# urgent-challenge/urgent2026_challenge_track1

Hardware: NVIDIA B200
Metric: BSRNN audio-sec/sec enhanced at 48 kHz (higher is better)
Workload: dtype fp16

## Files before the change

### include/bsrnn_b200.h

```cpp
#ifndef BSRNN_B200_H_
#define BSRNN_B200_H_

#include <stdint.h>
#include <stddef.h>

#ifdef __cplusplus
extern "C" {
#endif

const char* bsrnn_last_error(void);
int bsrnn_abi_version(void);
int bsrnn_device_check(void);
long bsrnn_launch_count(int reset);

int bsrnn_fft_twiddle(float* twiddle, int n_fft, void* stream);
int bsrnn_stft_fwd(const float* wav, const int32_t* lens, float* spec, const float* twiddle, int B, int L,
                   int n_fft, int hop, int transform, float exponent, float factor, void* stream);

int bsrnn_istft_fwd(const float* spec, const float* mask, const float* resid, float* spec_out, float* wav_out,
                    const float* twiddle, int B, int T, int L_out, int n_fft, int hop, int transform,
                    float exponent, float factor, void* stream);

int bsrnn_gn_stats(const float* x, double* stats, int B, long rows_per_sample, int C, long row_stride, void* stream);
int bsrnn_band_stats(const float* x, double* stats, int B, int T, long row_len, const int32_t* band_off,
                     const int32_t* band_width, int n_bands, void* stream);
int bsrnn_gn_finalize(const double* stats, const float* gamma, const float* beta, const float* extra,
                      float* scale, float* shift, int G, int C, const double* counts, float eps, int G_inner,
                      void* stream);

typedef struct {
  const float* A; const float* W; const float* bias; float* C;
  const float* scale; const float* shift;
  long a_inner, a_outer_stride, a_inner_stride;
  long c_inner, c_outer_stride, c_inner_stride;
  long rows_per_sample, ss_stride;
  int M, N, K, k_valid, ldw, epilogue, n_store, pad_;
} bsrnn_gemm_desc;
int bsrnn_gemm_f32(const bsrnn_gemm_desc* descs, int n_groups, int max_m, int max_n, void* stream);

int bsrnn_blstm_recurrence_f32(const float* gates_x, const float* w_hh, float* y, float* c_state,
                               int R, int steps, int H, long seq_inner, long seq_outer, long seq_inner_stride,
                               long step_stride, void* stream);

int bsrnn_norm_cast_kb8(const float* x, const float* scale, const float* shift, void* out, long ldx, int col0, int C,
                        int kcores, int m_tiles, int tiles_per_step, int R, long seq_inner, long seq_outer,
                        long seq_inner_stride, long step_stride, long tokens_per_sample, int g_inner, void* stream);
int bsrnn_norm_cast_kb8_ones(const float* x, const float* scale, const float* shift, void* out, long ldx, int col0,
                             int C, int kcores, int m_tiles, int tiles_per_step, int R, long seq_inner, long seq_outer,
                             long seq_inner_stride, long step_stride, long tokens_per_sample, int g_inner, int one_col,
                             void* stream);
int bsrnn_gemm_tc(const void* A, const void* W, const float* bias, void* out, double* stats, int m_tiles, int n_tiles,
                  int kcores, int BN, int epilogue, long ldo, int n_valid, int out_kcores, long tokens_per_sample,
                  int tiles_per_step, int R, long seq_inner, long seq_outer, long seq_inner_stride, long step_stride,
                  void* stream);
int bsrnn_gemm_tc_ex(const void* A, const void* W, const float* bias, void* out, double* stats, int m_tiles, int n_tiles,
                     int kcores, int BN, int epilogue, long ldo, int n_valid, int out_kcores, long tokens_per_sample,
                     int tiles_per_step, int R, long seq_inner, long seq_outer, long seq_inner_stride, long step_stride,
                     int stats_inner, int flags, void* stream);
int bsrnn_gemm_tc_grouped(const void* A, const void* W, const float* bias, void* out, double* stats,
                          const long long* groups, int n_groups, int m_tiles, int kc_max, int BN, long ldo, int n_valid,
                          long tokens_per_sample, int tiles_per_step, int R, long seq_inner, long seq_outer,
                          long seq_inner_stride, long step_stride, void* stream);
int bsrnn_gemm_tc_limit_ctas(int n);
int bsrnn_band_norm_cast_kb8(const float* spec, const float* scale, const float* shift, void* out, const int32_t* c_off,
                             const int32_t* bin0, const int32_t* width2, const long long* a_off, int K, long rows, int T,
                             int F2, int cmax, void* stream);
int bsrnn_lstm_step_tc(const void* A, const void* W, const void* gx, float* cstate, void* out_h, int m_tiles, int n_tiles,
                       int BN, int H, long ld_gx, void* stream);
int bsrnn_blstm_step_tc(const void* A_f, const void* W_f, const void* gx_f, float* c_f, void* out_f, const void* A_b,
                        const void* W_b, const void* gx_b, float* c_b, void* out_b, int m_tiles, int n_tiles, int BN,
                        int H, long ld_gx, void* stream);
int bsrnn_blstm_recurrence_tc(const void* gates_x, const void* w_pack, const void* zero_tile, void* y, int R, int steps,
                              int seq_tiles, int max_clusters, void* stream);
int bsrnn_blstm_recurrence_tc_ex(const void* gates_x, const void* w_pack, const void* zero_tile, void* y, int R,
                                 int steps, int seq_tiles, int max_clusters, int slots, void* stream);
int bsrnn_blstm_tc_max_clusters(void);
int bsrnn_blstm_tc_max_pair_clusters(void);
int bsrnn_blstm_recurrence_tc_flag(const void* gates_x, const void* w_pack, const void* zero_tile, void* y, int R,
                                   int steps, int seq_tiles, int max_groups, int slots, void* sync_ws, void* stream);
int bsrnn_blstm_tc_flag_max_groups(void);
int bsrnn_blstm_tc_sync_bytes(void);
int bsrnn_blstm_fused_tc(const void* xhat, const void* w_fused, const void* zero_tile, void* y, int R, int steps,
                         int seq_tiles, int max_groups, int slots, void* sync_ws, void* stream);
int bsrnn_blstm_fused_max_groups(void);
int bsrnn_blstm_fused_sync_bytes(void);
int bsrnn_blstm_fused7_tc(const void* xhat, const void* w_fused7, const void* zero_tile, void* y, int R, int steps,
                          int seq_tiles, int max_groups, int slots, void* sync_ws, void* stream);
int bsrnn_blstm_fused7_max_groups(void);
int bsrnn_blstm_fused14_tc(const void* xhat, const void* w_fused14, const void* zero_tile, void* y, int R, int steps,
                           int seq_tiles, int max_groups, int slots, void* sync_ws, void* stream);
int bsrnn_blstm_fused_train_tc(int geo, const void* xhat, const void* w_fused, const void* zero_tile, void* y_f, void* y_b,
                               long y_stride, void* gates, float* c_f, float* c_b, void* scratch, int R, int steps,
                               int seq_tiles, int max_groups, int slots, void* sync_ws, void* stream);
long bsrnn_blstm_fused_train_scratch_bytes(int steps, int seq_tiles);
int bsrnn_blstm_fused14_max_groups(void);
int bsrnn_blstm_fused768_tc(const void* xhat, const void* w_fused, const void* zero_tile, void* y_f, void* y_b,
                            long y_stride, int R, int steps, int seq_tiles, int max_groups, int slots, void* sync_ws,
                            void* stream);
int bsrnn_blstm_fused768_max_groups(void);

void bsrnn_debug_set_lstm_schedule(int ver);

int bsrnn_blstm_train_fwd_f32(const float* gates_x, const float* w_hh, float* y, float* c_state, float* saved, int R,
                              int steps, int H, long seq_inner, long seq_outer, long seq_inner_stride,
                              long step_stride, void* stream);
int bsrnn_blstm_train_bwd_f32(const float* dy, const float* saved, const float* w_hh, float* dgates, float* dh_rec,
                              float* dc_carry, int R, int steps, int H, long seq_inner, long seq_outer,
                              long seq_inner_stride, long step_stride, void* stream);
int bsrnn_grad_sumsq(const float* grad, long n, double* stats, void* stream);
int bsrnn_adamw_step(float* param, const float* grad, float* exp_avg, float* exp_avg_sq, float* ema, long n,
                     const double* stats, float grad_scale, float max_norm, float lr, float beta1, float beta2,
                     float eps, float weight_decay, int step, float ema_decay, void* stream);
int bsrnn_adamw_step2(float* param, const float* grad, float* exp_avg, float* exp_avg_sq, float* ema, long n,
                      double* state, const long* skip_ranges, int n_skip, float grad_scale, float max_norm, float lr,
                      float beta1, float beta2, float eps, float weight_decay, float ema_decay, void* stream);

int bsrnn_blstm_step_train_tc(const void* A_f, const void* W_f, void* gx_f, const float* cprev_f, float* cout_f, void* out_f,
                              const void* A_b, const void* W_b, void* gx_b, const float* cprev_b, float* cout_b,
                              void* out_b, int m_tiles, int n_tiles, int BN, int H, long ld_gx, void* stream);
int bsrnn_blstm_bwd_step_tc(const void* A_f, const void* W_f, const void* sg_f, const void* dy_f, const float* ccur_f,
                            const float* cprev_f, float* dc_f, void* out_f, const void* A_b, const void* W_b,
                            const void* sg_b, const void* dy_b, const float* ccur_b, const float* cprev_b, float* dc_b,
                            void* out_b, int m_tiles, int n_tiles, int BN, int H, long ld_sg, long ld_dy, int valid_rows,
                            void* stream);
int bsrnn_blstm_train_fwd_tc(const void* zero_tile, void* y_f, void* y_b, const void* W_f, const void* W_b, void* gates,
                             float* c_f, float* c_b, int steps, int tiles, int n_tiles, int BN, int H, void* stream);
int bsrnn_blstm_train_bwd_tc(const void* zero_tile, void* dG_f, void* dG_b, const void* WT_f, const void* WT_b,
                             const void* gates, const void* dy, const float* c_f, const float* c_b, float* dc_f, float* dc_b,
                             int steps, int tiles, int n_tiles, int BN, int H, int valid_rows, void* stream);
int bsrnn_gemm_tc_scaled(const void* A, const void* W, const float* bias, void* out, int m_tiles, int n_tiles, int kcores,
                         int BN, long ldo, int n_valid, float out_scale, const float* out_scale_ptr, int ksplit,
                         int tiles_per_step, int R, long seq_inner, long seq_outer, long seq_inner_stride,
                         long step_stride, void* stream);
int bsrnn_kb8_transpose(const void* src, void* dst, int src_m0, int m_count, int kc_src, int BN, int n_tiles,
                        long dst_kcores, long dst_kc0, void* stream);

int bsrnn_stft_stats_fwd(const float* wav, const int32_t* lens, float* spec, const float* twiddle, int B, int L, int n_fft,
                         int hop, int transform, float exponent, float factor, double* band_stats,
                         const int32_t* band_bin0, int n_bands, void* stream);
int bsrnn_band_split_fwd(const float* spec, const float* scale, const float* shift, const float* wT, const float* bias,
                         float* out, const int32_t* c_off, const int32_t* bin0, const int32_t* width2,
                         const int32_t* c_off_host, int K, long rows, int T, int F2, int N, int cmax, long ldo,
                         int out_width, int out_col, void* stream);

int bsrnn_istft_bwd(const float* d_wav, float* d_spec, const float* twiddle, int B, int T, int L_out, int n_fft, int hop,
                    void* stream);

int bsrnn_l1_time_fwd_bwd(const float* est, const float* tgt, double* loss, float* grad, int B, int L, float weight,
                          void* stream);
int bsrnn_mrl1_spec_fwd_bwd(const float* est, const float* tgt, double* loss, float* grad, const float* twiddle, int B,
                            int L, int window, float weight, void* stream);

int bsrnn_time_embed(const float* t, const float* W, float* out, int B, int E, void* stream);
int bsrnn_conv5x5_glu(const float* g, const float* weight, const float* bias, float* out, int B, int T, int Fp,
                      int F, void* stream);
int bsrnn_euler_step(float* x, const float* mask, const float* resid, float step, long n_complex, void* stream);
int bsrnn_axpy_complex(float* out, const float* y, const float* z, float sigma, long n_complex, void* stream);
int bsrnn_complex_mask(float* out, const float* x, const float* mask, const float* resid, float sign, long n_complex,
                       void* stream);

#ifdef __cplusplus
}
#endif
#endif
```

### urgent2026_challenge_track1_b200/_lib.py

```python
from __future__ import annotations

import ctypes as C
import os

import numpy as np
import torch

_HERE = os.path.dirname(os.path.abspath(__file__))
LIB_PATH = os.path.join(_HERE, "_C", "libbsrnn_b200.so")

c_void_p, c_int, c_long, c_float, c_double = C.c_void_p, C.c_int, C.c_long, C.c_float, C.c_double

PROTOTYPES = {
    "bsrnn_abi_version": [],
    "bsrnn_device_check": [],
    "bsrnn_launch_count": [c_int],
    "bsrnn_fft_twiddle": [c_void_p, c_int, c_void_p],
    "bsrnn_stft_fwd": [c_void_p, c_void_p, c_void_p, c_void_p, c_int, c_int, c_int, c_int, c_int, c_float, c_float,
                       c_void_p],
    "bsrnn_istft_fwd": [c_void_p, c_void_p, c_void_p, c_void_p, c_void_p, c_void_p, c_int, c_int, c_int, c_int,
                        c_int, c_int, c_float, c_float, c_void_p],
    "bsrnn_gn_stats": [c_void_p, c_void_p, c_int, c_long, c_int, c_long, c_void_p],
    "bsrnn_band_stats": [c_void_p, c_void_p, c_int, c_int, c_long, c_void_p, c_void_p, c_int, c_void_p],
    "bsrnn_gn_finalize": [c_void_p, c_void_p, c_void_p, c_void_p, c_void_p, c_void_p, c_int, c_int, c_void_p,
                          c_float, c_int, c_void_p],
    "bsrnn_gemm_f32": [c_void_p, c_int, c_int, c_int, c_void_p],
    "bsrnn_blstm_recurrence_f32": [c_void_p, c_void_p, c_void_p, c_void_p, c_int, c_int, c_int, c_long, c_long,
                                   c_long, c_long, c_void_p],
    "bsrnn_norm_cast_kb8": [c_void_p, c_void_p, c_void_p, c_void_p, c_long, c_int, c_int, c_int, c_int, c_int, c_int,
                            c_long, c_long, c_long, c_long, c_long, c_int, c_void_p],
    "bsrnn_norm_cast_kb8_ones": [c_void_p, c_void_p, c_void_p, c_void_p, c_long, c_int, c_int, c_int, c_int, c_int,
                                 c_int, c_long, c_long, c_long, c_long, c_long, c_int, c_int, c_void_p],
    "bsrnn_gemm_tc": [c_void_p, c_void_p, c_void_p, c_void_p, c_void_p, c_int, c_int, c_int, c_int, c_int, c_long,
                      c_int, c_int, c_long, c_int, c_int, c_long, c_long, c_long, c_long, c_void_p],
    "bsrnn_gemm_tc_ex": [c_void_p, c_void_p, c_void_p, c_void_p, c_void_p, c_int, c_int, c_int, c_int, c_int, c_long,
                         c_int, c_int, c_long, c_int, c_int, c_long, c_long, c_long, c_long, c_int, c_int, c_void_p],
    "bsrnn_gemm_tc_grouped": [c_void_p, c_void_p, c_void_p, c_void_p, c_void_p, c_void_p, c_int, c_int, c_int, c_int, c_long,
                              c_int, c_long, c_int, c_int, c_long, c_long, c_long, c_long, c_void_p],
    "bsrnn_gemm_tc_limit_ctas": [c_int],
    "bsrnn_blstm_fused_train_tc": [c_int, c_void_p, c_void_p, c_void_p, c_void_p, c_void_p, c_long, c_void_p, c_void_p, c_void_p,
                                   c_void_p, c_int, c_int, c_int, c_int, c_int, c_void_p, c_void_p],
    "bsrnn_blstm_fused_train_scratch_bytes": [c_int, c_int],
    "bsrnn_band_norm_cast_kb8": [c_void_p, c_void_p, c_void_p, c_void_p, c_void_p, c_void_p, c_void_p, c_void_p, c_int,
                                 c_long, c_int, c_int, c_int, c_void_p],
    "bsrnn_lstm_step_tc": [c_void_p, c_void_p, c_void_p, c_void_p, c_void_p, c_int, c_int, c_int, c_int, c_long, c_void_p],
    "bsrnn_blstm_step_tc": [c_void_p, c_void_p, c_void_p, c_void_p, c_void_p, c_void_p, c_void_p, c_void_p, c_void_p, c_void_p,
                            c_int, c_int, c_int, c_int, c_long, c_void_p],
    "bsrnn_blstm_recurrence_tc": [c_void_p, c_void_p, c_void_p, c_void_p, c_int, c_int, c_int, c_int, c_void_p],
    "bsrnn_blstm_recurrence_tc_ex": [c_void_p, c_void_p, c_void_p, c_void_p, c_int, c_int, c_int, c_int, c_int,
                                     c_void_p],
    "bsrnn_blstm_recurrence_tc_flag": [c_void_p, c_void_p, c_void_p, c_void_p, c_int, c_int, c_int, c_int, c_int,
                                       c_void_p, c_void_p],
    "bsrnn_blstm_fused_tc": [c_void_p, c_void_p, c_void_p, c_void_p, c_int, c_int, c_int, c_int, c_int, c_void_p, c_void_p],
    "bsrnn_blstm_fused768_tc": [c_void_p, c_void_p, c_void_p, c_void_p, c_void_p, c_long, c_int, c_int, c_int, c_int, c_int,
                                c_void_p, c_void_p],
    "bsrnn_blstm_fused768_max_groups": [],
    "bsrnn_blstm_fused7_tc": [c_void_p, c_void_p, c_void_p, c_void_p, c_int, c_int, c_int, c_int, c_int, c_void_p, c_void_p],
    "bsrnn_blstm_fused7_max_groups": [],
    "bsrnn_blstm_fused14_tc": [c_void_p, c_void_p, c_void_p, c_void_p, c_int, c_int, c_int, c_int, c_int, c_void_p, c_void_p],
    "bsrnn_blstm_fused14_max_groups": [],
    "bsrnn_blstm_fused_max_groups": [],
    "bsrnn_blstm_fused_sync_bytes": [],
    "bsrnn_blstm_tc_flag_max_groups": [],
    "bsrnn_blstm_tc_sync_bytes": [],
    "bsrnn_blstm_tc_max_clusters": [],
    "bsrnn_blstm_tc_max_pair_clusters": [],
    "bsrnn_debug_set_lstm_schedule": [c_int],
    "bsrnn_blstm_train_fwd_f32": [c_void_p, c_void_p, c_void_p, c_void_p, c_void_p, c_int, c_int, c_int, c_long, c_long,
                                  c_long, c_long, c_void_p],
    "bsrnn_blstm_train_bwd_f32": [c_void_p, c_void_p, c_void_p, c_void_p, c_void_p, c_void_p, c_int, c_int, c_int,
                                  c_long, c_long, c_long, c_long, c_void_p],
    "bsrnn_grad_sumsq": [c_void_p, c_long, c_void_p, c_void_p],
    "bsrnn_adamw_step": [c_void_p, c_void_p, c_void_p, c_void_p, c_void_p, c_long, c_void_p, c_float, c_float, c_float,
                         c_float, c_float, c_float, c_float, c_int, c_float, c_void_p],
    "bsrnn_adamw_step2": [c_void_p, c_void_p, c_void_p, c_void_p, c_void_p, c_long, c_void_p, c_void_p, c_int, c_float,
                          c_float, c_float, c_float, c_float, c_float, c_float, c_float, c_void_p],
    "bsrnn_blstm_step_train_tc": [c_void_p] * 12 + [c_int, c_int, c_int, c_int, c_long, c_void_p],
    "bsrnn_blstm_bwd_step_tc": [c_void_p] * 16 + [c_int, c_int, c_int, c_int, c_long, c_long, c_int, c_void_p],
    "bsrnn_blstm_train_fwd_tc": [c_void_p] * 8 + [c_int, c_int, c_int, c_int, c_int, c_void_p],
    "bsrnn_blstm_train_bwd_tc": [c_void_p] * 11 + [c_int, c_int, c_int, c_int, c_int, c_int, c_void_p],
    "bsrnn_gemm_tc_scaled": [c_void_p, c_void_p, c_void_p, c_void_p, c_int, c_int, c_int, c_int, c_long, c_int, c_float,
                             c_void_p, c_int, c_int, c_int, c_long, c_long, c_long, c_long, c_void_p],
    "bsrnn_kb8_transpose": [c_void_p, c_void_p, c_int, c_int, c_int, c_int, c_int, c_long, c_long, c_void_p],
    "bsrnn_stft_stats_fwd": [c_void_p, c_void_p, c_void_p, c_void_p, c_int, c_int, c_int, c_int, c_int, c_float, c_float,
                             c_void_p, c_void_p, c_int, c_void_p],
    "bsrnn_band_split_fwd": [c_void_p] * 10 + [c_int, c_long, c_int, c_int, c_int, c_int, c_long, c_int, c_int, c_void_p],
    "bsrnn_istft_bwd": [c_void_p, c_void_p, c_void_p, c_int, c_int, c_int, c_int, c_int, c_void_p],
    "bsrnn_l1_time_fwd_bwd": [c_void_p, c_void_p, c_void_p, c_void_p, c_int, c_int, c_float, c_void_p],
    "bsrnn_mrl1_spec_fwd_bwd": [c_void_p, c_void_p, c_void_p, c_void_p, c_void_p, c_int, c_int, c_int, c_float, c_void_p],
    "bsrnn_time_embed": [c_void_p, c_void_p, c_void_p, c_int, c_int, c_void_p],
    "bsrnn_conv5x5_glu": [c_void_p, c_void_p, c_void_p, c_void_p, c_int, c_int, c_int, c_int, c_void_p],
    "bsrnn_euler_step": [c_void_p, c_void_p, c_void_p, c_float, c_long, c_void_p],
    "bsrnn_axpy_complex": [c_void_p, c_void_p, c_void_p, c_float, c_long, c_void_p],
    "bsrnn_complex_mask": [c_void_p, c_void_p, c_void_p, c_void_p, c_float, c_long, c_void_p],
}

GEMM_DESC = np.dtype([
    ("A", "<u8"), ("W", "<u8"), ("bias", "<u8"), ("C", "<u8"), ("scale", "<u8"), ("shift", "<u8"),
    ("a_inner", "<i8"), ("a_outer_stride", "<i8"), ("a_inner_stride", "<i8"),
    ("c_inner", "<i8"), ("c_outer_stride", "<i8"), ("c_inner_stride", "<i8"),
    ("rows_per_sample", "<i8"), ("ss_stride", "<i8"),
    ("M", "<i4"), ("N", "<i4"), ("K", "<i4"), ("k_valid", "<i4"), ("ldw", "<i4"), ("epilogue", "<i4"),
    ("n_store", "<i4"), ("pad_", "<i4"),
])
assert GEMM_DESC.itemsize == 144

EPI_STORE, EPI_TANH, EPI_RESIDUAL, EPI_GLU = 0, 1, 2, 3
TC_F16_ROWS, TC_RESID_F32, TC_TANH_KB8, TC_GLU_F32, TC_F16_KB8 = 0, 1, 2, 3, 4
TC_TANH_F32 = 7
TC_RESID_TMA = 8

_lib = None


class NativeLibraryError(RuntimeError):
    pass


def lib():
    global _lib
    if _lib is None:
        if not os.path.exists(LIB_PATH):
            raise NativeLibraryError(
                f"{LIB_PATH} not found: the CUDA extension is not built (run ./build.sh). "
                "There is no CPU or PyTorch fallback for this path.")
        handle = C.CDLL(LIB_PATH)
        for name, argtypes in PROTOTYPES.items():
            fn = getattr(handle, name)
            fn.argtypes = argtypes
            fn.restype = c_int
        handle.bsrnn_launch_count.restype = C.c_long
        handle.bsrnn_blstm_fused_train_scratch_bytes.restype = C.c_long
        handle.bsrnn_last_error.restype = C.c_char_p
        handle.bsrnn_last_error.argtypes = []
        _lib = handle
    return _lib


def check(rc: int, what: str):
    if rc != 0:
        raise RuntimeError(f"{what} failed (rc={rc}): {lib().bsrnn_last_error().decode()}")


_DEVICE_OK = set()


def require_device():
    if not torch.cuda.is_available():
        raise NativeLibraryError("no CUDA device: the B200 path has no CPU fallback")
    dev = torch.cuda.current_device()
    if dev not in _DEVICE_OK:
        check(lib().bsrnn_device_check(), "bsrnn_device_check")
        _DEVICE_OK.add(dev)


def ptr(t):
    if t is None:
        return None
    return t.data_ptr()


def stream_ptr():
    return torch.cuda.current_stream().cuda_stream


def call(name, *args):
    check(getattr(lib(), name)(*args), name)
```

### urgent2026_challenge_track1_b200/csrc/gemm_tc.cu

```cuda
#include "common.cuh"
#include "umma.cuh"
#include "tmap.cuh"
#include <cuda_fp16.h>
#include <stdlib.h>

namespace bsrnn {
using namespace umma;

constexpr int TC_STAGES = 8;
constexpr int TC_KS = 8;
constexpr int TC_EPI_WARPS = 8;
#ifndef BSRNN_RESID_EPI_WARPS
#define BSRNN_RESID_EPI_WARPS 12
#endif
__host__ __device__ constexpr int tc_epi_warps(int epi) { return (epi == 1  || epi == 8 ) ? BSRNN_RESID_EPI_WARPS : TC_EPI_WARPS; }
__host__ __device__ constexpr int tc_threads(int epi) { return (2 + tc_epi_warps(epi)) * 32; }
constexpr int TC_SCR_LD = 36;
constexpr int TC_SCR_BYTES = tc_epi_warps(1) * 32 * TC_SCR_LD * 4;
constexpr int TC_ACC_COLS = 256;

struct RowMap {
  int tiles_per_step;
  int R;
  long seq_inner, seq_outer, seq_inner_stride, step_stride;
  __device__ __forceinline__ bool map(int m_tile, int r, long* token) const {
    const int step = m_tile / tiles_per_step;
    const int j = m_tile - step * tiles_per_step;
    const int seq = j * 128 + r;
    if (seq >= R) return false;
    if (seq_inner == 1) *token = (long)seq * seq_outer + (long)step * step_stride;
    else if (seq_inner >= (long)R) *token = (long)seq * seq_inner_stride + (long)step * step_stride;
    else {
      const int si = (int)seq_inner, q = seq / si;
      *token = (long)q * seq_outer + (long)(seq - q * si) * seq_inner_stride + (long)step * step_stride;
    }
    return true;
  }
};

struct GemmTcArgs {
  const __half* A;
  const __half* W;
  const float* bias;
  void* out;
  double* stats;
  long ldo;
  long tokens_per_sample;
  int m_tiles, n_tiles, kcores, BN;
  int n_valid;
  int out_kcores;
  int b_resident;
  int pf_dist;
  int ks;
  const __half* gx;
  float* cstate;
  long ld_gx;
  int H;
  int dir_tiles;
  const __half* A2; const __half* W2; const __half* gx2; float* cstate2; void* out2;
  int debug;
  int stages;
  RowMap rows;
  float out_scale;
  const float* out_scale_ptr;
  int ksplit, kps, m_log;
  int mc;
  int save_gates;
  float* cstate_out; float* cstate_out2;
  const __half* dy; const __half* dy2;
  long ld_dy;
  const float* c_cur; const float* c_cur2;
  const float* c_prev; const float* c_prev2;
  int valid_rows;
  alignas(64) CUtensorMap tmap;
  const long long* groups;
  int n_groups;
  int l2_keep;
  int reverse_m;
  int m_inner;
  int use_tmap;
  int tm_col_step;
  int run_merge;
  int no_resid;
  int stats_inner;
};

enum { EPI_F16_ROWS = 0, EPI_RESID_F32 = 1, EPI_TANH_KB8 = 2, EPI_GLU_F32 = 3, EPI_F16_KB8 = 4, EPI_LSTM_STEP = 5,
       EPI_LSTM_BWD = 6, EPI_TANH_F32 = 7, EPI_RESID_TMA = 8 };

__device__ __forceinline__ float fast_tanh(float x) {
  float y;
  asm("tanh.approx.f32 %0, %1;" : "=f"(y) : "f"(x));
  return y;
}
__device__ __forceinline__ float fast_sigmoid(float x) { return fmaf(fast_tanh(0.5f * x), 0.5f, 0.5f); }

__device__ __forceinline__ uint32_t pack_h2(float a, float b) {
  __half2 v = __floats2half2_rn(a, b);
  return *reinterpret_cast<uint32_t*>(&v);
}

struct BwdSub {
  uint4 g[4];
  uint4 dy;
  float4 cc[2], cq[2], dc[2];
};
__device__ __forceinline__ void bwd_load(BwdSub& R, const __half* sgp, const __half* dyp, const float* ccp, const float* cpp,
                                         const float* dcp, int b8) {
#pragma unroll
  for (int i = 0; i < 4; ++i) R.g[i] = __ldg(reinterpret_cast<const uint4*>(sgp + 32 * b8) + i);
  R.dy = __ldg(reinterpret_cast<const uint4*>(dyp + 8 * b8));
  R.cc[0] = __ldg(reinterpret_cast<const float4*>(ccp + 8 * b8));
  R.cc[1] = __ldg(reinterpret_cast<const float4*>(ccp + 8 * b8 + 4));
  R.cq[0] = R.cq[1] = make_float4(0.f, 0.f, 0.f, 0.f);
  if (cpp) {
    R.cq[0] = __ldg(reinterpret_cast<const float4*>(cpp + 8 * b8));
    R.cq[1] = __ldg(reinterpret_cast<const float4*>(cpp + 8 * b8 + 4));
  }
  R.dc[0] = *reinterpret_cast<const float4*>(dcp + 8 * b8);
  R.dc[1] = *reinterpret_cast<const float4*>(dcp + 8 * b8 + 4);
}
__device__ __forceinline__ void bwd_unit(float dh_rec, float dy, float i_, float f_, float g_, float o_, float ct, float cprev,
                                         float& dc_carry, uint32_t& w0, uint32_t& w1) {
  const float dh = dy + dh_rec;
  const float tc = fast_tanh(ct);
  const float d_o = dh * tc;
  const float dc = dc_carry + dh * o_ * (1.f - tc * tc);
  const float d_i = dc * g_, d_g = dc * i_, d_f = dc * cprev;
  dc_carry = dc * f_;
  w0 = pack_h2(d_i * i_ * (1.f - i_), d_f * f_ * (1.f - f_));
  w1 = pack_h2(d_g * (1.f - g_ * g_), d_o * o_ * (1.f - o_));
}
__device__ __forceinline__ void bwd_compute(BwdSub& R, float a0, float a1, float a2, float a3, float a4, float a5, float a6,
                                            float a7, uint32_t (&dgw)[16]) {
  const __half2* gh = reinterpret_cast<const __half2*>(R.g);
  const __half2* dyh = reinterpret_cast<const __half2*>(&R.dy);
  const float acc[8] = {a0, a1, a2, a3, a4, a5, a6, a7};
  const float ct[8] = {R.cc[0].x, R.cc[0].y, R.cc[0].z, R.cc[0].w, R.cc[1].x, R.cc[1].y, R.cc[1].z, R.cc[1].w};
  const float cp[8] = {R.cq[0].x, R.cq[0].y, R.cq[0].z, R.cq[0].w, R.cq[1].x, R.cq[1].y, R.cq[1].z, R.cq[1].w};
  float dcs[8] = {R.dc[0].x, R.dc[0].y, R.dc[0].z, R.dc[0].w, R.dc[1].x, R.dc[1].y, R.dc[1].z, R.dc[1].w};
#pragma unroll
  for (int j = 0; j < 8; ++j) {
    const float2 g_if = __half22float2(gh[2 * j]), g_go = __half22float2(gh[2 * j + 1]);
    const float2 d2 = __half22float2(dyh[j >> 1]);
    bwd_unit(acc[j], (j & 1) ? d2.y : d2.x, g_if.x, g_if.y, g_go.x, g_go.y, ct[j], cp[j], dcs[j], dgw[2 * j], dgw[2 * j + 1]);
  }
  R.dc[0] = make_float4(dcs[0], dcs[1], dcs[2], dcs[3]);
  R.dc[1] = make_float4(dcs[4], dcs[5], dcs[6], dcs[7]);
}

template <int EPI, int NC>
__device__ __forceinline__ void epilogue_chunk(const GemmTcArgs& a, int m, int n, int r, int c0, const uint32_t* acc,
                                               bool row_ok, long token, float& s_sum, float& s_sq, float* scr, int lane,
                                               float bias_lane) {
  const int gc0 = n * a.BN + c0;
  float v[NC];
  if (a.bias) {
#pragma unroll
    for (int i = 0; i < NC; ++i) v[i] = __uint_as_float(acc[i]) + __shfl_sync(0xffffffffu, bias_lane, i);
  } else {
#pragma unroll
    for (int i = 0; i < NC; ++i) v[i] = __uint_as_float(acc[i]);
  }
  if (EPI == EPI_RESID_F32 && (a.out_scale != 0.f || a.out_scale_ptr)) {
    const float sc = a.out_scale_ptr ? __ldg(a.out_scale_ptr) : a.out_scale;
#pragma unroll
    for (int i = 0; i < NC; ++i) v[i] *= sc;
  }

  if (EPI == EPI_F16_ROWS) {
    if (!row_ok) return;
    __half* o = reinterpret_cast<__half*>(a.out) + token * a.ldo + gc0;
#pragma unroll
    for (int i = 0; i < NC; i += 8) {
      uint4 pk = make_uint4(pack_h2(v[i], v[i + 1]), pack_h2(v[i + 2], v[i + 3]), pack_h2(v[i + 4], v[i + 5]),
                            pack_h2(v[i + 6], v[i + 7]));
      *reinterpret_cast<uint4*>(o + i) = pk;
    }
  } else if (EPI == EPI_RESID_F32) {
    if (a.debug & 4) return;
    float* my = scr + (r & 31) * TC_SCR_LD;
#pragma unroll
    for (int i = 0; i < NC; i += 4) *reinterpret_cast<float4*>(my + i) = make_float4(v[i], v[i + 1], v[i + 2], v[i + 3]);
    __syncwarp();
    const int sub = lane >> 3, c4 = (lane & 7) * 4;
    const unsigned okmask = __ballot_sync(0xffffffffu, row_ok);
    const bool col_ok = c4 < NC && gc0 + c4 + 3 < a.n_valid;
    float* optr[8];
    float4 old[8];
#pragma unroll
    for (int i = 0; i < 8; ++i) {
      const int rr = 4 * i + sub;
      const long tok = __shfl_sync(0xffffffffu, token, rr);
      optr[i] = (((okmask >> rr) & 1u) && col_ok) ? reinterpret_cast<float*>(a.out) + tok * a.ldo + gc0 + c4 : nullptr;
      old[i] = make_float4(0.f, 0.f, 0.f, 0.f);
      if (optr[i] && a.ksplit <= 1 && !(a.debug & 8)) old[i] = *reinterpret_cast<const float4*>(optr[i]);
    }
    if (a.ksplit > 1) {
#pragma unroll
      for (int i = 0; i < 8; ++i) {
        if (optr[i]) {
          const float4 nv = *reinterpret_cast<const float4*>(scr + (4 * i + sub) * TC_SCR_LD + c4);
          atomicAdd(optr[i], nv.x); atomicAdd(optr[i] + 1, nv.y); atomicAdd(optr[i] + 2, nv.z); atomicAdd(optr[i] + 3, nv.w);
        }
      }
      __syncwarp();
      return;
    }
#pragma unroll
    for (int i = 0; i < 8; ++i) {
      if (optr[i]) {
        float* sp = scr + (4 * i + sub) * TC_SCR_LD + c4;
        float4 nv = *reinterpret_cast<const float4*>(sp);
        nv.x += old[i].x; nv.y += old[i].y; nv.z += old[i].z; nv.w += old[i].w;
        *reinterpret_cast<float4*>(optr[i]) = nv;
        *reinterpret_cast<float4*>(sp) = nv;
      }
    }
    __syncwarp();
    if (row_ok && a.stats && !(a.debug & 16)) {
#pragma unroll
      for (int i = 0; i < NC; i += 4) {
        if (gc0 + i + 3 < a.n_valid) {
          const float4 nv = *reinterpret_cast<const float4*>(my + i);
          s_sum += nv.x + nv.y + nv.z + nv.w;
          s_sq += nv.x * nv.x + nv.y * nv.y + nv.z * nv.z + nv.w * nv.w;
        }
      }
    }
    __syncwarp();
  } else if (EPI == EPI_F16_KB8) {
    __half* o = reinterpret_cast<__half*>(a.out) + (((long)m * a.out_kcores + (gc0 >> 3)) * 128 + r) * 8;
#pragma unroll
    for (int i = 0; i < NC; i += 8) {
      uint4 pk = make_uint4(pack_h2(v[i], v[i + 1]), pack_h2(v[i + 2], v[i + 3]), pack_h2(v[i + 4], v[i + 5]),
                            pack_h2(v[i + 6], v[i + 7]));
      *reinterpret_cast<uint4*>(o + (long)(i >> 3) * 1024) = pk;
    }
  } else if (EPI == EPI_LSTM_STEP) {
    if (NC == 32) {
      const int u0 = gc0 >> 2;
      if (u0 < a.H) {
        const bool dir2 = a.dir_tiles > 0 && m >= a.dir_tiles;
        const int md = dir2 ? m - a.dir_tiles : m;
        const long grow = (long)md * 128 + r;
        const uint4* gp = reinterpret_cast<const uint4*>((dir2 ? a.gx2 : a.gx) + grow * a.ld_gx + gc0);
        const float* cin = dir2 ? a.cstate2 : a.cstate;
        float* cout = dir2 ? a.cstate_out2 : a.cstate_out;
        const float* cp = cin ? cin + grow * a.H + u0 : nullptr;
        float* cpo = cout ? cout + grow * a.H + u0 : const_cast<float*>(cp);
        uint4 g4[4];
        if (a.save_gates) {
#pragma unroll
          for (int i = 0; i < 4; ++i) g4[i] = gp[i];
        } else {
#pragma unroll
          for (int i = 0; i < 4; ++i) g4[i] = __ldg(gp + i);
        }
        float4 c4[2] = {make_float4(0.f, 0.f, 0.f, 0.f), make_float4(0.f, 0.f, 0.f, 0.f)};
        if (cp) { c4[0] = *reinterpret_cast<const float4*>(cp); c4[1] = *reinterpret_cast<const float4*>(cp + 4); }
        float* c = reinterpret_cast<float*>(c4);
        const __half2* gh = reinterpret_cast<const __half2*>(g4);
        float h[8];
        uint32_t sv[16];
#pragma unroll
        for (int j = 0; j < 8; ++j) {
          const float2 g01 = __half22float2(gh[2 * j]), g23 = __half22float2(gh[2 * j + 1]);
          const float ig = fmaf(fast_tanh(v[4 * j] + g01.x), 0.5f, 0.5f), fg = fmaf(fast_tanh(v[4 * j + 1] + g01.y), 0.5f, 0.5f);
          const float gg = fast_tanh(v[4 * j + 2] + g23.x), og = fmaf(fast_tanh(v[4 * j + 3] + g23.y), 0.5f, 0.5f);
          c[j] = fmaf(fg, c[j], ig * gg);
          h[j] = og * fast_tanh(c[j]);
          sv[2 * j] = pack_h2(ig, fg);
          sv[2 * j + 1] = pack_h2(gg, og);
        }
        if (a.save_gates) {
          uint4* gw = const_cast<uint4*>(gp);
#pragma unroll
          for (int i = 0; i < 4; ++i) gw[i] = make_uint4(sv[4 * i], sv[4 * i + 1], sv[4 * i + 2], sv[4 * i + 3]);
        }
        *reinterpret_cast<float4*>(cpo) = c4[0];
        *reinterpret_cast<float4*>(cpo + 4) = c4[1];
        __half* o = reinterpret_cast<__half*>(dir2 ? a.out2 : a.out) + (((long)md * a.out_kcores + (u0 >> 3)) * 128 + r) * 8;
        *reinterpret_cast<uint4*>(o) = make_uint4(pack_h2(h[0], h[1]), pack_h2(h[2], h[3]), pack_h2(h[4], h[5]), pack_h2(h[6], h[7]));
      }
    }
  } else if (EPI == EPI_LSTM_BWD) {
    if (NC == 32) {
      const int u0 = gc0;
      if (u0 < a.H) {
        const bool dir2 = a.dir_tiles > 0 && m >= a.dir_tiles;
        const int md = dir2 ? m - a.dir_tiles : m;
        const long grow = (long)md * 128 + r;
        const bool live = grow < a.valid_rows;
        const __half* sgp = (dir2 ? a.gx2 : a.gx) + grow * a.ld_gx + 4 * u0;
        const __half* dyp = (dir2 ? a.dy2 : a.dy) + grow * a.ld_dy + u0;
        const float* ccp = (dir2 ? a.c_cur2 : a.c_cur) + grow * a.H + u0;
        const float* cpv = dir2 ? a.c_prev2 : a.c_prev;
        const float* cpp = cpv ? cpv + grow * a.H + u0 : nullptr;
        float* dcp = (dir2 ? a.cstate2 : a.cstate) + grow * a.H + u0;
        __half* o = reinterpret_cast<__half*>(dir2 ? a.out2 : a.out) + (((long)md * a.out_kcores + (u0 >> 1)) * 128 + r) * 8;
        BwdSub ra;
#pragma unroll
        for (int b8 = 0; b8 < 4; ++b8) {
          if (u0 + 8 * b8 >= a.H) break;
          uint32_t dgw[16];
          if (live) {
            bwd_load(ra, sgp, dyp, ccp, cpp, dcp, b8);
            bwd_compute(ra, v[8 * b8], v[8 * b8 + 1], v[8 * b8 + 2], v[8 * b8 + 3], v[8 * b8 + 4], v[8 * b8 + 5], v[8 * b8 + 6],
                        v[8 * b8 + 7], dgw);
            *reinterpret_cast<float4*>(dcp + 8 * b8) = ra.dc[0];
            *reinterpret_cast<float4*>(dcp + 8 * b8 + 4) = ra.dc[1];
          } else {
#pragma unroll
            for (int i = 0; i < 16; ++i) dgw[i] = 0u;
          }
#pragma unroll
          for (int i = 0; i < 4; ++i)
            *reinterpret_cast<uint4*>(o + (size_t)(4 * b8 + i) * 1024) = make_uint4(dgw[4 * i], dgw[4 * i + 1], dgw[4 * i + 2], dgw[4 * i + 3]);
        }
      }
    }
  } else if (EPI == EPI_TANH_KB8) {
    __half* o = reinterpret_cast<__half*>(a.out);
#pragma unroll
    for (int i = 0; i < NC; i += 8) {
      const int kc = (gc0 + i) >> 3;
      if (kc >= a.out_kcores) break;
      float t[8];
#pragma unroll
      for (int j = 0; j < 8; ++j) t[j] = (gc0 + i + j < a.n_valid) ? fast_tanh(v[i + j]) : 0.f;
      uint4 pk = make_uint4(pack_h2(t[0], t[1]), pack_h2(t[2], t[3]), pack_h2(t[4], t[5]), pack_h2(t[6], t[7]));
      *reinterpret_cast<uint4*>(o + (((long)m * a.out_kcores + kc) * 128 + r) * 8) = pk;
    }
  } else if (EPI == EPI_TANH_F32) {
    if (!row_ok) return;
    float* o = reinterpret_cast<float*>(a.out) + token * a.ldo + gc0;
#pragma unroll
    for (int i = 0; i < NC; i += 4)
      if (gc0 + i + 3 < a.n_valid)
        *reinterpret_cast<float4*>(o + i) = make_float4(fast_tanh(v[i]), fast_tanh(v[i + 1]), fast_tanh(v[i + 2]), fast_tanh(v[i + 3]));
  } else if (EPI == EPI_GLU_F32) {
    if (!row_ok) return;
    float* o = reinterpret_cast<float*>(a.out) + token * a.ldo + (gc0 >> 1);
#pragma unroll
    for (int i = 0; i < NC; i += 2)
      if (((gc0 + i) >> 1) < a.n_valid) o[i >> 1] = v[i] * fast_sigmoid(v[i + 1]);
  }
}

struct TileIter {
  int m, n;
  int dm, dn, n_tiles, m_tiles;
  bool resident;
  __device__ __forceinline__ TileIter(const GemmTcArgs& a) {
    n_tiles = a.n_tiles; m_tiles = a.m_tiles; resident = a.b_resident != 0;
    if (resident && a.dir_tiles > 0) {
      const int nt2 = 2 * n_tiles;
      const int vn = (int)blockIdx.x % nt2;
      const int dir = vn / n_tiles;
      n = vn - dir * n_tiles;
      dm = (int)gridDim.x / nt2;
      m = dir * a.dir_tiles + (int)blockIdx.x / nt2;
      m_tiles = dir == 0 ? a.dir_tiles : a.m_tiles;
      dn = 0;
      return;
    }
    n = (int)blockIdx.x % n_tiles;
    m = (int)blockIdx.x / n_tiles;
    dm = (int)gridDim.x / n_tiles;
    dn = resident ? 0 : (int)gridDim.x - dm * n_tiles;
    if (a.reverse_m && n_tiles == 1 && !resident) {
      rev = true;
      m = m_tiles - 1 - (int)blockIdx.x;
      dm = -(int)gridDim.x;
    } else if (a.m_inner > 1 && !resident && dn == 0) {
      inner = a.m_inner; tps = a.rows.tiles_per_step;
      lin = m;
      m = (lin % inner) * tps + lin / inner;
    }
  }
  bool rev = false;
  int inner = 0, tps = 0, lin = 0;
  __device__ __forceinline__ bool valid() const { return rev ? m >= 0 : (inner ? lin < m_tiles : m < m_tiles); }
  __device__ __forceinline__ void next() {
    if (inner) {
      lin += dm;
      m = (lin % inner) * tps + lin / inner;
      return;
    }
    m += dm; n += dn;
    if (n >= n_tiles) { n -= n_tiles; ++m; }
  }
  __device__ __forceinline__ TileIter ahead(int k) const {
    TileIter t = *this;
    for (int i = 0; i < k; ++i) t.next();
    return t;
  }
};

template <int NCORES>
__device__ __forceinline__ void store_kb8_cores(__half* o, const uint32_t (&v)[32]) {
#pragma unroll
  for (int i = 0; i < NCORES; ++i) {
    const uint4 pk = make_uint4(pack_h2(__uint_as_float(v[8 * i]), __uint_as_float(v[8 * i + 1])),
                                pack_h2(__uint_as_float(v[8 * i + 2]), __uint_as_float(v[8 * i + 3])),
                                pack_h2(__uint_as_float(v[8 * i + 4]), __uint_as_float(v[8 * i + 5])),
                                pack_h2(__uint_as_float(v[8 * i + 6]), __uint_as_float(v[8 * i + 7])));
    *reinterpret_cast<uint4*>(o + (size_t)i * 1024) = pk;
  }
}

template <int NCORES>
__device__ __forceinline__ void store_kb8_cores_smem(uint8_t* p, const uint32_t (&v)[32]) {
#pragma unroll
  for (int i = 0; i < NCORES; ++i) {
    const uint4 pk = make_uint4(pack_h2(__uint_as_float(v[8 * i]), __uint_as_float(v[8 * i + 1])),
                                pack_h2(__uint_as_float(v[8 * i + 2]), __uint_as_float(v[8 * i + 3])),
                                pack_h2(__uint_as_float(v[8 * i + 4]), __uint_as_float(v[8 * i + 5])),
                                pack_h2(__uint_as_float(v[8 * i + 6]), __uint_as_float(v[8 * i + 7])));
    *reinterpret_cast<uint4*>(p + (size_t)i * 2048) = pk;
  }
}
__device__ __forceinline__ void named_bar_sync(int id, int nthreads) {
  asm volatile("bar.sync %0, %1;" ::"r"(id), "r"(nthreads) : "memory");
}

template <int EPI, int BNC = 0>
__global__ void __launch_bounds__(tc_threads(EPI), 1) gemm_tc_kernel(const __grid_constant__ GemmTcArgs a) {
  extern __shared__ __align__(128) uint8_t smem[];
  const int BN = a.BN;
  const int KS = a.ks;
  const uint32_t a_stage_bytes = KS * 128 * 16;
  const uint32_t b_stage_bytes = KS * BN * 16;
  uint8_t* sA = smem;
  const uint32_t NST = (uint32_t)a.stages;
  uint8_t* sB = smem + NST * a_stage_bytes;
  const uint32_t b_region = a.b_resident ? (uint32_t)a.kcores * BN * 16 : NST * b_stage_bytes;
  uint64_t* bars = reinterpret_cast<uint64_t*>(sB + b_region);
  uint64_t* full = bars;
  uint64_t* empty = bars + TC_STAGES;
  uint64_t* acc_full = bars + 2 * TC_STAGES;
  uint64_t* acc_empty = bars + 2 * TC_STAGES + 2;
  uint64_t* b_full = bars + 2 * TC_STAGES + 4;
  uint64_t* res_full = bars + 2 * TC_STAGES + 5;
  uint32_t* tmem_slot = reinterpret_cast<uint32_t*>(bars + 2 * TC_STAGES + 6);
  uint8_t* smem_scr = reinterpret_cast<uint8_t*>(bars + 2 * TC_STAGES + 8);

  const int warp = threadIdx.x >> 5, lane = threadIdx.x & 31;
  if (threadIdx.x == 0) {
    for (int i = 0; i < TC_STAGES; ++i) { mbar_init(full + i, 1); mbar_init(empty + i, a.mc > 1 ? a.mc : 1); }
    for (int i = 0; i < 2; ++i) { mbar_init(acc_full + i, 1); mbar_init(acc_empty + i, BNC ? TC_EPI_WARPS / 2 : tc_epi_warps(EPI)); }
    mbar_init(b_full, 1);
    mbar_init(res_full, 128);
    fence_barrier_init();
  }
  if (warp == 2) tmem_alloc(tmem_slot, 2 * TC_ACC_COLS);
  tc_fence_before();
  __syncthreads();
  if (a.mc > 1) cluster_sync();
  tc_fence_after();
  const uint32_t tmem_base = *tmem_slot;
  const uint32_t crank = a.mc > 1 ? cluster_ctarank() : 0u;
  const uint16_t cmask = (uint16_t)((1u << (a.mc > 1 ? a.mc : 1)) - 1u);

  if (warp == 0) {
    if (elect_one()) {
      uint32_t stage = 0, phase = 0;
      TileIter ti(a);
      int pf_mod = 0, pf_dmod = 0;
      if (a.b_resident && a.pf_dist > 0) {
        const TileIter t3 = ti.ahead(a.pf_dist);
        pf_mod = t3.m % a.n_tiles; pf_dmod = ti.dm % a.n_tiles;
      }
      if (a.b_resident && ti.valid()) {
        const uint8_t* gB = reinterpret_cast<const uint8_t*>((a.dir_tiles > 0 && ti.m >= a.dir_tiles) ? a.W2 : a.W) +
                            (size_t)ti.n * a.kcores * BN * 16;
        const uint32_t bytes = (uint32_t)a.kcores * BN * 16;
        mbar_expect_tx(b_full, bytes);
        for (uint32_t off = 0; off < bytes; off += 32768) bulk_g2s(sB + off, gB + off, min(32768u, bytes - off), b_full);
      }
      for (; ti.valid(); ti.next()) {
        const bool dir2 = a.dir_tiles > 0 && ti.m >= a.dir_tiles;
        const int split = a.ksplit > 1 ? ti.m / a.m_log : 0;
        const int mrow = dir2 ? ti.m - a.dir_tiles : (a.ksplit > 1 ? ti.m - split * a.m_log : ti.m);
        const int kbase = split * a.kps;
        int kcnt = a.ksplit > 1 ? min(a.kps, a.kcores - kbase) : a.kcores;
        const uint8_t* gA = reinterpret_cast<const uint8_t*>(dir2 ? a.A2 : a.A) + ((size_t)mrow * a.kcores + kbase) * 2048;
        const uint8_t* gB = reinterpret_cast<const uint8_t*>(dir2 ? a.W2 : a.W) + ((size_t)ti.n * a.kcores + kbase) * BN * 16;
        if (a.groups) {
          const long long* G = a.groups + 5 * (ti.m % a.n_groups);
          kcnt = (int)__ldg(G + 4);
          gA = reinterpret_cast<const uint8_t*>(a.A + __ldg(G)) + (size_t)(ti.m / a.n_groups) * kcnt * 2048;
          gB = reinterpret_cast<const uint8_t*>(a.W + __ldg(G + 1));
        }
        const int nstage_t = (kcnt + KS - 1) / KS;
        if (a.pf_dist > 0) {
          const TileIter t3 = ti.ahead(a.pf_dist);
          if (t3.valid() && (a.b_resident ? ti.n == pf_mod : t3.n == 0))
            bulk_prefetch_l2(reinterpret_cast<const uint8_t*>(a.A) + (size_t)t3.m * a.kcores * 2048, (uint32_t)a.kcores * 2048);
          pf_mod += pf_dmod;
          if (pf_mod >= a.n_tiles) pf_mod -= a.n_tiles;
        }
        for (int ks = 0; ks < nstage_t; ++ks) {
          const int kc0 = ks * KS;
          const int nk = min(KS, kcnt - kc0);
          mbar_wait(empty + stage, phase ^ 1);
          mbar_expect_tx(full + stage, (uint32_t)nk * (2048 + (a.b_resident ? 0 : BN * 16)));
          if (a.mc > 1) {
            const uint32_t slice = (uint32_t)nk * 2048 / (uint32_t)a.mc;
            bulk_g2s_multicast(sA + stage * a_stage_bytes + crank * slice, gA + (size_t)kc0 * 2048 + crank * slice, slice,
                               full + stage, cmask);
          } else if (a.l2_keep & 2)
            bulk_g2s_hint(sA + stage * a_stage_bytes, gA + (size_t)kc0 * 2048, nk * 2048, full + stage, l2_policy_evict_last());
          else
          bulk_g2s(sA + stage * a_stage_bytes, gA + (size_t)kc0 * 2048, nk * 2048, full + stage);
          if (!a.b_resident)
            bulk_g2s(sB + stage * b_stage_bytes, gB + (size_t)kc0 * BN * 16, nk * BN * 16, full + stage);
          if (++stage == NST) { stage = 0; phase ^= 1; }
        }
      }
    }
  } else if (warp == 1) {
    if (elect_one()) {
      const uint32_t idesc = idesc_f16_f32(128, BN);
      TileIter ti(a);
      if (a.b_resident && ti.valid()) mbar_wait(b_full, 0);
      const uint64_t da0 = smem_desc_kb8(smem_u32(sA), 2048, 128);
      const uint64_t db0 = smem_desc_kb8(smem_u32(sB), BN * 16, 128);
      const uint32_t a_step = (2 * 2048) >> 4, b_step = (uint32_t)(2 * BN * 16) >> 4;
      {
        uint32_t stage = 0, phase = 0;
        for (int it = 0; ti.valid(); ti.next(), ++it) {
          const int buf = it & 1;
          const uint32_t acc_phase = (it >> 1) & 1;
          mbar_wait(acc_empty + buf, acc_phase ^ 1);
          tc_fence_after();
          const uint32_t d_tmem = tmem_base + buf * TC_ACC_COLS;
          const int kcnt = a.groups ? (int)__ldg(a.groups + 5 * (ti.m % a.n_groups) + 4)
                                    : (a.ksplit > 1 ? min(a.kps, a.kcores - (ti.m / a.m_log) * a.kps) : a.kcores);
          const int nstage_t = (kcnt + KS - 1) / KS;
          for (int ks = 0; ks < nstage_t; ++ks) {
            const int nk = min(KS, kcnt - ks * KS);
            mbar_wait(full + stage, phase);
            tc_fence_after();
            const uint64_t da = da0 + (uint64_t)(stage * (a_stage_bytes >> 4));
            const uint64_t db = db0 + (uint64_t)(a.b_resident ? (uint32_t)ks * (KS / 2) * b_step : stage * (b_stage_bytes >> 4));
            for (int j = 0; j < nk / 2; ++j) mma_f16_ss(d_tmem, da + (uint64_t)(j * a_step), db + (uint64_t)(j * b_step), idesc, (ks | j) != 0);
            if (a.mc > 1) mma_commit_multicast(empty + stage, cmask);
            else mma_commit(empty + stage);
            if (++stage == NST) { stage = 0; phase ^= 1; }
          }
          mma_commit(acc_full + buf);
        }
      }
    }
  } else {
    const int q = warp & 3;
    const int half = (warp - 2) >> 2;
    const int r = q * 32 + lane;
    if constexpr ((EPI == EPI_F16_KB8 || EPI == EPI_TANH_KB8) && BNC == 208) {
      const int n = blockIdx.x % a.n_tiles;
      const int mstep = gridDim.x / a.n_tiles;
      constexpr uint32_t STG_BYTES = 14 * 2048;
      uint8_t* stg = smem_scr + half * STG_BYTES;
      uint8_t* my_stg = stg + r * 16;
      uint8_t* gbase = reinterpret_cast<uint8_t*>(a.out) + (size_t)(n * (BNC / 8)) * 2048;
      const size_t o_tile = (a.debug & 1) ? 0 : (size_t)a.out_kcores * 2048;
      const bool do_store = !(a.debug & 2);
      const bool leader = (warp == 2 + 4 * half) && lane == 0;
      const uint32_t t_row = tmem_base + half * TC_ACC_COLS + ((uint32_t)(q * 32) << 16);
      const int bar_id = 1 + half;
      const int cores_left = a.out_kcores - n * (BNC / 8);
      const uint32_t nA = (uint32_t)(cores_left < 14 ? (cores_left < 0 ? 0 : cores_left) : 14);
      constexpr int NB_MAX = EPI == EPI_TANH_KB8 ? 12 : 11;
      const uint32_t nB = (uint32_t)(cores_left - 14 < 0 ? 0 : (cores_left - 14 > NB_MAX ? NB_MAX : cores_left - 14));
      auto act = [](uint32_t (&v)[32], int cnt) {
        if constexpr (EPI == EPI_TANH_KB8) {
#pragma unroll
          for (int i = 0; i < 32; ++i)
            if (i < cnt) v[i] = __float_as_uint(fast_tanh(__uint_as_float(v[i])));
        }
      };
      uint32_t acc_phase = 0;
      for (int m = blockIdx.x / a.n_tiles + half * mstep; m < a.m_tiles; m += 2 * mstep, acc_phase ^= 1) {
        uint32_t v0[32], v1[32], v2[32], v3[32];
        uint8_t* gdst = gbase + (size_t)m * o_tile;
        mbar_wait(acc_full + half, acc_phase);
        tc_fence_after();
        tmem_ld_x32(t_row, v0);
        tmem_ld_x32(t_row + 32, v1);
        tmem_ld_x32(t_row + 64, v2);
        tmem_ld_x16(t_row + 96, reinterpret_cast<uint32_t(&)[16]>(v3));
        tmem_ld_wait();
        tmem_ld_pin(v0); tmem_ld_pin(v1); tmem_ld_pin(v2); tmem_ld_pin(v3);
        act(v0, 32); act(v1, 32); act(v2, 32); act(v3, 16);
        if (leader) bulk_store_wait_read();
        named_bar_sync(bar_id, 128);
        store_kb8_cores_smem<4>(my_stg, v0);
        store_kb8_cores_smem<4>(my_stg + 4 * 2048, v1);
        store_kb8_cores_smem<4>(my_stg + 8 * 2048, v2);
        store_kb8_cores_smem<2>(my_stg + 12 * 2048, v3);
        fence_proxy_async_shared();
        named_bar_sync(bar_id, 128);
        if (leader && do_store && nA) {
          if (EPI == EPI_TANH_KB8 && (a.l2_keep & 1)) bulk_s2g_hint(gdst, stg, nA * 2048, l2_policy_evict_last());
          else bulk_s2g(gdst, stg, nA * 2048);
        }
        tmem_ld_x32(t_row + 112, v0);
        tmem_ld_x32(t_row + 144, v1);
        tmem_ld_x32(t_row + 176, v2);
        tmem_ld_wait();
        tmem_ld_pin(v0); tmem_ld_pin(v1); tmem_ld_pin(v2);
        tc_fence_before();
        __syncwarp();
        if (lane == 0) mbar_arrive(acc_empty + half);
        act(v0, 32); act(v1, 32); act(v2, 32);
        if (leader) bulk_store_wait_read();
        named_bar_sync(bar_id, 128);
        store_kb8_cores_smem<4>(my_stg, v0);
        store_kb8_cores_smem<4>(my_stg + 4 * 2048, v1);
        if constexpr (EPI == EPI_TANH_KB8) store_kb8_cores_smem<4>(my_stg + 8 * 2048, v2);
        else store_kb8_cores_smem<3>(my_stg + 8 * 2048, v2);
        fence_proxy_async_shared();
        named_bar_sync(bar_id, 128);
        if (leader && do_store && nB) {
          if (EPI == EPI_TANH_KB8 && (a.l2_keep & 1)) bulk_s2g_hint(gdst + 14 * 2048, stg, nB * 2048, l2_policy_evict_last());
          else bulk_s2g(gdst + 14 * 2048, stg, nB * 2048);
        }
      }
      if (leader) bulk_store_wait_all();
    } else if constexpr (EPI == EPI_RESID_TMA) {
      constexpr int NPART = tc_epi_warps(EPI) / 4;
      const int nch = (BN + 31) >> 5;
      const int ch0 = (half * nch) / NPART, ch1 = ((half + 1) * nch) / NPART;
      float* resbuf = reinterpret_cast<float*>((reinterpret_cast<uintptr_t>(smem_scr) + 127) & ~(uintptr_t)127);
      const int ncmax = a.n_valid < BN ? a.n_valid : BN;
      const int ldr = (ncmax % 8 == 4) ? ncmax : ncmax + 4;
      const bool loader = half == 0;
      float* myrow = resbuf + (size_t)r * ldr;
      auto run_rows = [&](bool ok, long tok) -> uint32_t {
        if (!a.run_merge) return ok ? 1u : 0u;
        const long ptok = __shfl_up_sync(0xffffffffu, tok, 1);
        const bool pok = __shfl_up_sync(0xffffffffu, ok ? 1 : 0, 1) != 0;
        const bool head = ok && (lane == 0 || !pok || tok != ptok + 1);
        const unsigned heads = __ballot_sync(0xffffffffu, head), oks = __ballot_sync(0xffffffffu, ok);
        if (!head) return 0u;
        const unsigned above = lane == 31 ? 0u : ((heads | ~oks) & ~((2u << lane) - 1u));
        return (uint32_t)((above ? __ffs(above) - 1 : 32) - lane);
      };
      auto issue_loads = [&](const TileIter& t) {
        const int m2 = t.m, n2 = t.n;
        long tok2 = 0;
        const int nc2 = (a.n_valid - n2 * BN < BN ? a.n_valid - n2 * BN : BN);
        if (a.use_tmap) {
          if (r == 0 && !a.no_resid) {
            const int step2 = m2 / a.rows.tiles_per_step;
            mbar_expect_tx(res_full, 128u * (uint32_t)nc2 * 4);
            tma_load_2d(resbuf, &a.tmap, step2 * a.tm_col_step + n2 * BN, (m2 - step2 * a.rows.tiles_per_step) * 128, res_full);
          } else {
            mbar_arrive(res_full);
          }
          return;
        }
        const bool ok2 = !a.no_resid && a.rows.map(m2, r, &tok2) && nc2 > 0;
        const uint32_t nr = run_rows(ok2, tok2);
        if (nr) {
          mbar_expect_tx(res_full, nr * (uint32_t)nc2 * 4);
          bulk_g2s(myrow, reinterpret_cast<const float*>(a.out) + tok2 * a.ldo + (long)n2 * BN, nr * (uint32_t)nc2 * 4, res_full);
        } else {
          mbar_arrive(res_full);
        }
      };
      TileIter ti(a);
      if (loader && ti.valid()) issue_loads(ti);
      for (int it = 0; ti.valid(); ti.next(), ++it) {
        const int m = a.groups ? ti.m / a.n_groups : ti.m, n = ti.n;
        const float* g_bias = a.bias;
        float* g_out = reinterpret_cast<float*>(a.out);
        int tm_col = 0;
        if (a.groups) {
          const long long* G = a.groups + 5 * (ti.m % a.n_groups);
          tm_col = (int)__ldg(G + 2);
          g_out += tm_col;
          if (g_bias) g_bias += __ldg(G + 3);
        }
        const int buf = it & 1;
        const uint32_t acc_phase = (it >> 1) & 1;
        long token = 0;
        const bool row_ok = a.rows.map(m, r, &token);
        const int ncols = (a.n_valid - n * BN < BN ? a.n_valid - n * BN : BN);
        float s_sum = 0.f, s_sq = 0.f;
        const TileIter tn = ti.ahead(1);
        {
          long tok2 = 0;
          if (!a.no_resid && tn.valid() && a.rows.map(tn.m, r, &tok2)) {
            const char* p = reinterpret_cast<const char*>(reinterpret_cast<const float*>(a.out) + tok2 * a.ldo + (long)tn.n * BN);
            const int nbytes = (a.n_valid - tn.n * BN < BN ? a.n_valid - tn.n * BN : BN) * 4;
            for (int off = half * 128; off < nbytes; off += NPART * 128) asm volatile("prefetch.global.L2 [%0];" ::"l"(p + off));
          }
        }
        float bl[4] = {0.f, 0.f, 0.f, 0.f};
        if (a.bias) {
#pragma unroll
          for (int i = 0; i < 4; ++i) {
            const int c = (ch0 + i) * 32 + lane;
            if (ch0 + i < ch1 && c < BN) bl[i] = __ldg(g_bias + n * BN + c);
          }
        }
        const float osc = a.out_scale_ptr ? __ldg(a.out_scale_ptr) : (a.out_scale != 0.f ? a.out_scale : 1.f);
        mbar_wait(acc_full + buf, acc_phase);
        tc_fence_after();
        mbar_wait(res_full, (uint32_t)(it & 1));
        const uint32_t t_addr = tmem_base + buf * TC_ACC_COLS + ((uint32_t)(q * 32) << 16);
#pragma unroll
        for (int i = 0; i < 4; ++i) {
          const int ch = ch0 + i;
          if (ch >= ch1) break;
          const int c0 = ch * 32;
          uint32_t acc[32];
          const bool wide = c0 + 32 <= BN;
          if (wide) tmem_ld_x32(t_addr + c0, acc);
          else tmem_ld_x16(t_addr + c0, reinterpret_cast<uint32_t(&)[16]>(acc));
          tmem_ld_wait();
          tmem_ld_pin(acc);
          const int nc = wide ? 32 : 16;
#pragma unroll
          for (int j = 0; j < 32; j += 4) {
            if (j >= nc || c0 + j + 3 >= ncols) continue;
            const float b0 = a.bias ? __shfl_sync(0xffffffffu, bl[i], j) : 0.f, b1 = a.bias ? __shfl_sync(0xffffffffu, bl[i], j + 1) : 0.f;
            const float b2 = a.bias ? __shfl_sync(0xffffffffu, bl[i], j + 2) : 0.f, b3 = a.bias ? __shfl_sync(0xffffffffu, bl[i], j + 3) : 0.f;
            if (row_ok) {
              float4 o = a.no_resid ? make_float4(0.f, 0.f, 0.f, 0.f) : *reinterpret_cast<float4*>(myrow + c0 + j);
              o.x += (__uint_as_float(acc[j]) + b0) * osc; o.y += (__uint_as_float(acc[j + 1]) + b1) * osc;
              o.z += (__uint_as_float(acc[j + 2]) + b2) * osc; o.w += (__uint_as_float(acc[j + 3]) + b3) * osc;
              *reinterpret_cast<float4*>(myrow + c0 + j) = o;
              s_sum += o.x + o.y + o.z + o.w;
              s_sq += o.x * o.x + o.y * o.y + o.z * o.z + o.w * o.w;
            }
          }
        }
        tc_fence_before();
        __syncwarp();
        if (lane == 0) mbar_arrive(acc_empty + buf);
        fence_proxy_async_shared();
        named_bar_sync(3, tc_epi_warps(EPI) * 32);
        if (loader) {
          if (a.use_tmap) {
            if (r == 0) {
              const int step = m / a.rows.tiles_per_step;
              tma_store_2d(&a.tmap, tm_col + step * a.tm_col_step + n * BN, (m - step * a.rows.tiles_per_step) * 128, resbuf);
            }
          } else {
          const uint32_t nr = run_rows(row_ok && ncols > 0, token);
          if (nr) bulk_s2g(g_out + token * a.ldo + (long)n * BN, myrow, nr * (uint32_t)ncols * 4);
          }
          bulk_store_wait_read();
          named_bar_sync(4, 128);
          if (tn.valid()) issue_loads(tn);
        }
        if (a.stats) {
          const long samp = row_ok ? (a.stats_inner > 1 ? (token / a.tokens_per_sample) * a.stats_inner + token % a.stats_inner : token / a.tokens_per_sample) : -1;
          unsigned todo = __ballot_sync(0xffffffffu, row_ok);
          while (todo) {
            const int leader = __ffs(todo) - 1;
            const long ls = __shfl_sync(0xffffffffu, samp, leader);
            const bool mine = row_ok && samp == ls;
            const float ps = warp_sum(mine ? s_sum : 0.f);
            const float pq = warp_sum(mine ? s_sq : 0.f);
            if (lane == leader) {
              atomicAdd(a.stats + 2 * ls, (double)ps);
              atomicAdd(a.stats + 2 * ls + 1, (double)pq);
            }
            todo &= ~__ballot_sync(0xffffffffu, mine);
          }
        }
      }
      if (loader) bulk_store_wait_all();
    } else {
    const int nch = (BN + 31) >> 5;
    constexpr int NPART = tc_epi_warps(EPI) / 4;
    const int ch0 = (half * nch + NPART - 1) / NPART, ch1 = ((half + 1) * nch + NPART - 1) / NPART;
    float* scr = reinterpret_cast<float*>(smem_scr) + (warp - 2) * 32 * TC_SCR_LD;
    TileIter ti(a);
    for (int it = 0; ti.valid(); ti.next(), ++it) {
      const int m = a.ksplit > 1 ? ti.m % a.m_log : ti.m, n = ti.n;
      const int buf = it & 1;
      const uint32_t acc_phase = (it >> 1) & 1;
      long token = 0;
      const bool row_ok = a.rows.map(m, r, &token);
      float s_sum = 0.f, s_sq = 0.f;
      if (EPI == EPI_RESID_F32) {
        const TileIter t2 = ti.ahead(1);
        const int m2 = a.ksplit > 1 ? t2.m % a.m_log : t2.m, n2 = t2.n;
        long tok2 = 0;
        if (t2.valid() && a.rows.map(m2, r, &tok2)) {
          const char* p = reinterpret_cast<const char*>(reinterpret_cast<const float*>(a.out) + tok2 * a.ldo + n2 * a.BN);
          const int nbytes = (a.n_valid - n2 * a.BN < a.BN ? a.n_valid - n2 * a.BN : a.BN) * 4;
          for (int off = half * 128; off < nbytes; off += NPART * 128) asm volatile("prefetch.global.L2 [%0];" ::"l"(p + off));
        }
      }
      float bl[4] = {0.f, 0.f, 0.f, 0.f};
      if (a.bias) {
#pragma unroll
        for (int i = 0; i < 4; ++i) {
          const int c = (ch0 + i) * 32 + lane;
          if (ch0 + i < ch1 && c < BN) bl[i] = __ldg(a.bias + n * BN + c);
        }
      }
      mbar_wait(acc_full + buf, acc_phase);
      tc_fence_after();
      const uint32_t t_addr = tmem_base + buf * TC_ACC_COLS + ((uint32_t)(q * 32) << 16);
      uint32_t acc0[32], acc1[32];
      auto issue = [&](int ch, uint32_t (&dst)[32]) {
        const int c0 = ch * 32;
        if (c0 + 32 <= BN) tmem_ld_x32(t_addr + c0, dst);
        else tmem_ld_x16(t_addr + c0, reinterpret_cast<uint32_t(&)[16]>(dst));
      };
      auto consume = [&](int ch, int i, uint32_t (&src)[32]) {
        const int c0 = ch * 32;
        tmem_ld_pin(src);
        if (c0 + 32 <= BN) epilogue_chunk<EPI, 32>(a, m, n, r, c0, src, row_ok, token, s_sum, s_sq, scr, lane, bl[i]);
        else epilogue_chunk<EPI, 16>(a, m, n, r, c0, src, row_ok, token, s_sum, s_sq, scr, lane, bl[i]);
      };
      if constexpr (EPI == EPI_RESID_F32 && tc_epi_warps(EPI) > 8) {
#pragma unroll
        for (int i = 0; i < 4; ++i) {
          const int ch = ch0 + i;
          if (ch >= ch1) break;
          issue(ch, acc0);
          tmem_ld_wait();
          consume(ch, i, acc0);
        }
      } else {
      if (ch0 < ch1) issue(ch0, acc0);
#pragma unroll
      for (int i = 0; i < 4; ++i) {
        const int ch = ch0 + i;
        if (ch >= ch1) break;
        tmem_ld_wait();
        if ((i & 1) == 0) {
          if (ch + 1 < ch1) issue(ch + 1, acc1);
          consume(ch, i, acc0);
        } else {
          if (ch + 1 < ch1) issue(ch + 1, acc0);
          consume(ch, i, acc1);
        }
      }
      }
      tc_fence_before();
      __syncwarp();
      if (lane == 0) mbar_arrive(acc_empty + buf);
      if (EPI == EPI_RESID_F32 && a.stats) {
        const long samp = row_ok ? (a.stats_inner > 1 ? (token / a.tokens_per_sample) * a.stats_inner + token % a.stats_inner : token / a.tokens_per_sample) : -1;
        unsigned todo = __ballot_sync(0xffffffffu, row_ok);
        while (todo) {
          const int leader = __ffs(todo) - 1;
          const long ls = __shfl_sync(0xffffffffu, samp, leader);
          const bool mine = row_ok && samp == ls;
          const float ps = warp_sum(mine ? s_sum : 0.f);
          const float pq = warp_sum(mine ? s_sq : 0.f);
          if (lane == leader) {
            atomicAdd(a.stats + 2 * ls, (double)ps);
            atomicAdd(a.stats + 2 * ls + 1, (double)pq);
          }
          todo &= ~__ballot_sync(0xffffffffu, mine);
        }
      }
    }
    }
  }
  tc_fence_before();
  __syncthreads();
  if (a.mc > 1) cluster_sync();
  if (warp == 2) {
    tc_fence_after();
    tmem_dealloc(tmem_base, 2 * TC_ACC_COLS);
  }
}

static size_t tc_smem_bytes(int BN, int kcores, bool resident, bool scratch, int stages, int ksz = TC_KS, size_t extra = 0) {
  const size_t b = resident ? (size_t)kcores * BN * 16 : (size_t)stages * ksz * BN * 16;
  return (size_t)stages * ksz * 128 * 16 + b + (2 * TC_STAGES + 8) * 8 + (scratch ? TC_SCR_BYTES : 0) + extra;
}
static size_t tc_resbuf_bytes(int BN, int n_valid) {
  const int nc = n_valid < BN ? n_valid : BN;
  const int ldr = (nc % 8 == 4) ? nc : nc + 4;
  return (size_t)128 * ldr * 4;
}

static int g_cta_limit = 0;

static bool tanh_bulk_enabled() {
  static int v = -1;
  if (v < 0) { const char* e = getenv("BSRNN_TANH_BULK"); v = (e && e[0] == '0') ? 0 : 1; }
  return v != 0;
}

template <int EPI>
static int launch_tc(GemmTcArgs a, cudaStream_t st) {
  static int sms = 0;
  if (sms == 0) {
    int dev = 0;
    cudaGetDevice(&dev);
    if (cudaDeviceGetAttribute(&sms, cudaDevAttrMultiProcessorCount, dev) != cudaSuccess || sms <= 0) sms = 148;
  }
  a.b_resident = (a.n_tiles > 1 && a.n_tiles <= sms && (size_t)a.kcores * a.BN * 16 <= 120 * 1024 &&
                  a.m_tiles >= 2 * (sms / a.n_tiles) && a.ksplit <= 1 && a.dir_tiles == 0) ? 1 : 0;
  int step_mc = 1;
  if (EPI == EPI_LSTM_STEP && a.n_tiles > 1) {
    static int res_env = -1, mc_env = -1;
    if (res_env < 0) { const char* e = getenv("BSRNN_STEP_RESIDENT"); res_env = (e && e[0] == '1') ? 1 : 0; }
    if (mc_env < 0) { const char* e = getenv("BSRNN_STEP_MC"); mc_env = (e && (e[0] == '1' || e[0] == '2' || e[0] == '4')) ? e[0] - '0' : 4; }
    const int ndir = a.dir_tiles > 0 ? 2 : 1;
    const int nt_all = a.n_tiles * ndir;
    const int per_dir = a.dir_tiles > 0 ? a.dir_tiles : a.m_tiles;
    if (res_env && nt_all <= sms && tc_smem_bytes(a.BN, a.kcores, true, false, 4) <= 227 * 1024 && per_dir >= 2 * (sms / nt_all) &&
        (a.dir_tiles == 0 || a.m_tiles == 2 * a.dir_tiles)) {
      a.b_resident = 1;
      if (mc_env > 1 && a.n_tiles % mc_env == 0) step_mc = mc_env;
    }
  }
  if (EPI == EPI_GLU_F32) {
    static int rev_env = -1;
    if (rev_env < 0) { const char* e = getenv("BSRNN_GLU_REVERSE"); rev_env = (e && e[0] == '0') ? 0 : 1; }
    a.reverse_m = rev_env;
  }
  if (EPI == EPI_TANH_KB8 || EPI == EPI_GLU_F32) {
    static int keep_env = -1;
    if (keep_env < 0) { const char* e = getenv("BSRNN_HIDDEN_L2"); keep_env = (e && e[0] == '1') ? 1 : 0; }
    a.l2_keep = keep_env ? (EPI == EPI_TANH_KB8 ? 1 : 2) : 0;
  }
  const size_t extra_smem = EPI == EPI_RESID_TMA ? tc_resbuf_bytes(a.BN, a.n_valid) + 128 : 0;
  if (EPI == EPI_RESID_TMA) {
    static int tmap_env = -1;
    if (tmap_env < 0) { const char* e = getenv("BSRNN_FC_TMAP"); tmap_env = (e && e[0] == '0') ? 0 : 1; }
    long row_stride = 0, col_step = 0;
    if (a.rows.seq_inner == 1) { row_stride = a.rows.seq_outer * a.ldo; col_step = a.rows.step_stride * a.ldo; }
    else if (a.rows.seq_inner >= (long)a.rows.R) { row_stride = a.rows.seq_inner_stride * a.ldo; col_step = a.rows.step_stride * a.ldo; }
    const long steps = (a.groups ? a.m_tiles / a.n_groups : a.m_tiles) / a.rows.tiles_per_step;
    a.use_tmap = 0;
    if (tmap_env && a.n_tiles == 1 && a.n_valid <= a.BN && a.n_valid % 8 == 4 && row_stride > 0 && a.ksplit <= 1 &&
        a.out_scale == 0.f && a.out_scale_ptr == nullptr && (steps - 1) * col_step + a.n_valid <= row_stride &&
        (!a.groups || col_step == 0) && col_step < (1L << 30) &&
        make_tmap_2d_f32(&a.tmap, a.out, (uint64_t)row_stride, (uint64_t)a.rows.R, (uint64_t)row_stride * 4, (uint32_t)a.n_valid, 128)) {
      a.use_tmap = 1;
      a.tm_col_step = (int)col_step;
      static int inner_env = -1;
      if (inner_env < 0) { const char* e = getenv("BSRNN_FC_BAND_INNER"); inner_env = (e && e[0] == '0') ? 0 : 1; }
      if (inner_env && !a.groups && steps > 1 && col_step > 0 && a.m_tiles == steps * a.rows.tiles_per_step) a.m_inner = (int)steps;
    }
  }
  if (EPI == EPI_RESID_TMA && !a.use_tmap) {
    static int runs_env = -1;
    if (runs_env < 0) { const char* e = getenv("BSRNN_FC_RUNS"); runs_env = (e && e[0] == '0') ? 0 : 1; }
    a.run_merge = (runs_env && a.n_tiles == 1 && a.n_valid <= a.BN && a.ldo == a.n_valid && a.n_valid % 8 == 4) ? 1 : 0;
  }
  a.stages = tc_smem_bytes(a.BN, a.kcores, a.b_resident, EPI == EPI_RESID_F32, 8, TC_KS, extra_smem) <= 227 * 1024 ? 8 : 4;
  while (a.stages > 2 && tc_smem_bytes(a.BN, a.kcores, a.b_resident, EPI == EPI_RESID_F32, a.stages, TC_KS, extra_smem) > 227 * 1024) --a.stages;
  static int force4 = -1;
  if (force4 < 0) { const char* e = getenv("BSRNN_GEMM_STAGES"); force4 = (e && e[0] == '4') ? 1 : 0; }
  if (force4) a.stages = 4;
  a.ks = TC_KS;
  static int ks_env = -1;
  if (ks_env < 0) { const char* e = getenv("BSRNN_GEMM_KS"); ks_env = (e && e[0] == '4') ? 4 : 8; }
  if (ks_env == 4 && a.stages == 4 && !a.b_resident && a.mc <= 1 && a.ksplit <= 1 && a.kcores >= 32 && a.kcores % 4 == 0 &&
      tc_smem_bytes(a.BN, a.kcores, false, EPI == EPI_RESID_F32, 8, 4, extra_smem) <= 227 * 1024) {
    a.ks = 4;
    a.stages = 8;
  }
  a.pf_dist = a.b_resident ? 3 : 0;
  static int dbg = -1;
  if (dbg < 0) { const char* e = getenv("BSRNN_GEMM_DEBUG"); dbg = (e && e[0] >= '0' && e[0] <= '9') ? atoi(e) : 0; }
  a.debug = dbg;
  static int pfd = -2;
  if (pfd == -2) { const char* e = getenv("BSRNN_GEMM_PFDIST"); pfd = (e && e[0] >= '0' && e[0] <= '9') ? e[0] - '0' : -1; }
  if (pfd >= 0) a.pf_dist = pfd;
  const size_t smem = tc_smem_bytes(a.BN, a.kcores, a.b_resident, EPI == EPI_RESID_F32, a.stages, a.ks, extra_smem);
  static size_t smem_set = 0;
  if (smem > smem_set) {
    BSRNN_CUDA_OK(cudaFuncSetAttribute(gemm_tc_kernel<EPI>, cudaFuncAttributeMaxDynamicSharedMemorySize, (int)smem));
    smem_set = smem;
  }
  const int total = a.m_tiles * a.n_tiles;
  const int sms_use = (g_cta_limit > 0 && g_cta_limit < sms) ? g_cta_limit : sms;
  int grid = total < sms_use ? total : sms_use;
  if (a.b_resident) {
    const int nt_all = a.n_tiles * (a.dir_tiles > 0 ? 2 : 1);
    grid = (sms_use / nt_all) * nt_all;
    if (grid < nt_all) grid = nt_all;
    if (a.dir_tiles > 0) a.pf_dist = 0;
  }
  if (EPI == EPI_F16_KB8 && a.BN == 208 && a.kcores == 26 && a.bias == nullptr && a.b_resident &&
      a.out_kcores >= a.n_tiles * 26) {
    a.stages = 5;
    const size_t smem_ip = tc_smem_bytes(a.BN, a.kcores, true, false, a.stages) + 2 * 14 * 2048;
    BSRNN_CUDA_OK(cudaFuncSetAttribute(gemm_tc_kernel<EPI_F16_KB8, 208>, cudaFuncAttributeMaxDynamicSharedMemorySize, (int)smem_ip));
    static int mc_env = -1;
    if (mc_env < 0) { const char* e = getenv("BSRNN_GEMM_MC"); mc_env = (e && (e[0] == '1' || e[0] == '2' || e[0] == '4')) ? e[0] - '0' : 1; }
    int mc = mc_env;
    if (mc > 1 && (a.n_tiles % mc != 0 || a.m_tiles < 2 * (sms / a.n_tiles))) mc = 1;
    if (mc > 1) {
      cudaLaunchConfig_t cfg = {};
      cfg.gridDim = dim3(grid); cfg.blockDim = dim3(tc_threads(EPI)); cfg.dynamicSmemBytes = smem_ip; cfg.stream = st;
      cudaLaunchAttribute at[1];
      at[0].id = cudaLaunchAttributeClusterDimension;
      at[0].val.clusterDim.x = mc; at[0].val.clusterDim.y = 1; at[0].val.clusterDim.z = 1;
      cfg.attrs = at; cfg.numAttrs = 1;
      static int max_cl[5] = {0, 0, 0, 0, 0};
      if (max_cl[mc] == 0) {
        int n = 0;
        if (cudaOccupancyMaxActiveClusters(&n, gemm_tc_kernel<EPI_F16_KB8, 208>, &cfg) != cudaSuccess || n <= 0) { cudaGetLastError(); n = -1; }
        max_cl[mc] = n;
      }
      if (max_cl[mc] > 0) {
        const int groups = (max_cl[mc] * mc) / a.n_tiles;
        if (groups >= 1) {
          if (groups * a.n_tiles < grid) grid = groups * a.n_tiles;
          cfg.gridDim = dim3(grid);
          a.mc = mc;
          BSRNN_CUDA_OK(cudaLaunchKernelEx(&cfg, gemm_tc_kernel<EPI_F16_KB8, 208>, a));
          BSRNN_LAUNCH_OK();
          return 0;
        }
      }
    }
    a.mc = 1;
    gemm_tc_kernel<EPI_F16_KB8, 208><<<grid, tc_threads(EPI_F16_KB8), smem_ip, st>>>(a);
  } else if (EPI == EPI_TANH_KB8 && a.BN == 208 && a.kcores == 26 && a.bias == nullptr && a.b_resident &&
             a.out_kcores > (a.n_tiles - 1) * 26 && tanh_bulk_enabled()) {
    a.stages = 5;
    a.mc = 1;
    const size_t smem_ip = tc_smem_bytes(a.BN, a.kcores, true, false, a.stages) + 2 * 14 * 2048;
    BSRNN_CUDA_OK(cudaFuncSetAttribute(gemm_tc_kernel<EPI_TANH_KB8, 208>, cudaFuncAttributeMaxDynamicSharedMemorySize, (int)smem_ip));
    gemm_tc_kernel<EPI_TANH_KB8, 208><<<grid, tc_threads(EPI_TANH_KB8), smem_ip, st>>>(a);
  } else if (step_mc > 1) {
    cudaLaunchConfig_t cfg = {};
    cfg.gridDim = dim3(grid); cfg.blockDim = dim3(tc_threads(EPI)); cfg.dynamicSmemBytes = smem; cfg.stream = st;
    cudaLaunchAttribute at[1];
    at[0].id = cudaLaunchAttributeClusterDimension;
    at[0].val.clusterDim.x = step_mc; at[0].val.clusterDim.y = 1; at[0].val.clusterDim.z = 1;
    cfg.attrs = at; cfg.numAttrs = 1;
    static int max_cl = 0;
    static size_t max_cl_smem = 0;
    if (max_cl == 0 || smem > max_cl_smem) {
      int n = 0;
      if (cudaOccupancyMaxActiveClusters(&n, gemm_tc_kernel<EPI>, &cfg) != cudaSuccess || n <= 0) { cudaGetLastError(); n = -1; }
      max_cl = n; max_cl_smem = smem;
    }
    const int nt_all = a.n_tiles * (a.dir_tiles > 0 ? 2 : 1);
    const int groups = max_cl > 0 ? (max_cl * step_mc) / nt_all : 0;
    if (groups >= 1) {
      if (groups * nt_all < grid) grid = groups * nt_all;
      cfg.gridDim = dim3(grid);
      a.mc = step_mc;
      BSRNN_CUDA_OK(cudaLaunchKernelEx(&cfg, gemm_tc_kernel<EPI>, a));
    } else {
      a.mc = 1;
      gemm_tc_kernel<EPI><<<grid, tc_threads(EPI), smem, st>>>(a);
    }
  } else {
    gemm_tc_kernel<EPI><<<grid, tc_threads(EPI), smem, st>>>(a);
  }
  BSRNN_LAUNCH_OK();
  return 0;
}

}
using namespace bsrnn;

extern "C" int bsrnn_gemm_tc_ex(const void* A, const void* W, const float* bias, void* out, double* stats,
                                  int m_tiles, int n_tiles, int kcores, int BN, int epilogue, long ldo, int n_valid,
                                  int out_kcores, long tokens_per_sample, int tiles_per_step, int R, long seq_inner,
                                  long seq_outer, long seq_inner_stride, long step_stride, int stats_inner, int flags,
                                  void* stream) {
  BSRNN_CHECK_ARG(A && W && out, "gemm_tc: null pointer");
  BSRNN_CHECK_ARG(m_tiles > 0 && n_tiles > 0 && kcores > 0 && kcores % 2 == 0, "gemm_tc: bad tile counts (kcores=%d)", kcores);
  BSRNN_CHECK_ARG(BN >= 16 && BN <= 256 && BN % 16 == 0, "gemm_tc: BN=%d must be a multiple of 16 in [16,256]", BN);
  BSRNN_CHECK_ARG(tiles_per_step > 0 && seq_inner > 0 && tokens_per_sample > 0, "gemm_tc: bad row map");
  BSRNN_CHECK_ARG((epilogue != EPI_RESID_F32 && epilogue != EPI_TANH_F32 && epilogue != EPI_RESID_TMA) || (n_valid % 4 == 0 && ldo % 4 == 0),
                  "gemm_tc: the f32-row epilogues need n_valid and ldo to be multiples of 4 (got %d, %ld)", n_valid, ldo);
  GemmTcArgs a{};
  a.A = reinterpret_cast<const __half*>(A);
  a.W = reinterpret_cast<const __half*>(W);
  a.bias = bias; a.out = out; a.stats = stats; a.ldo = ldo; a.tokens_per_sample = tokens_per_sample;
  a.m_tiles = m_tiles; a.n_tiles = n_tiles; a.kcores = kcores; a.BN = BN; a.n_valid = n_valid; a.out_kcores = out_kcores;
  a.rows = RowMap{tiles_per_step, R, seq_inner, seq_outer, seq_inner_stride, step_stride};
  BSRNN_CHECK_ARG(stats_inner >= 1 && (flags & ~1) == 0 && (!(flags & 1) || epilogue == EPI_RESID_TMA),
                  "gemm_tc: bad stats_inner / flags (store-only needs epilogue 8)");
  a.stats_inner = stats_inner;
  a.no_resid = flags & 1;
  cudaStream_t st = (cudaStream_t)stream;
  switch (epilogue) {
    case EPI_F16_ROWS: return launch_tc<EPI_F16_ROWS>(a, st);
    case EPI_RESID_F32: return launch_tc<EPI_RESID_F32>(a, st);
    case EPI_TANH_KB8: return launch_tc<EPI_TANH_KB8>(a, st);
    case EPI_GLU_F32: return launch_tc<EPI_GLU_F32>(a, st);
    case EPI_F16_KB8: return launch_tc<EPI_F16_KB8>(a, st);
    case EPI_TANH_F32: return launch_tc<EPI_TANH_F32>(a, st);
    case EPI_RESID_TMA:
      BSRNN_CHECK_ARG(BN % 4 == 0 && (reinterpret_cast<uintptr_t>(out) & 15) == 0, "gemm_tc: the TMA residual epilogue needs 16-byte aligned rows");
      return launch_tc<EPI_RESID_TMA>(a, st);
  }
  set_error("gemm_tc: unknown epilogue %d", epilogue);
  return 1;
}
extern "C" int bsrnn_gemm_tc_limit_ctas(int n) {
  const int prev = g_cta_limit;
  g_cta_limit = n > 0 ? n : 0;
  return prev;
}

extern "C" int bsrnn_gemm_tc_grouped(const void* A, const void* W, const float* bias, void* out, double* stats,
                                       const long long* groups, int n_groups, int m_tiles, int kc_max, int BN, long ldo,
                                       int n_valid, long tokens_per_sample, int tiles_per_step, int R, long seq_inner,
                                       long seq_outer, long seq_inner_stride, long step_stride, void* stream) {
  BSRNN_CHECK_ARG(A && W && out && groups && n_groups > 0, "gemm_tc_grouped: null pointer");
  BSRNN_CHECK_ARG(m_tiles > 0 && kc_max > 0 && kc_max % 2 == 0 && BN >= 16 && BN <= 256 && BN % 16 == 0, "gemm_tc_grouped: bad tile dims");
  BSRNN_CHECK_ARG(n_valid > 0 && n_valid <= BN && n_valid % 4 == 0 && ldo % 4 == 0 && (reinterpret_cast<uintptr_t>(out) & 15) == 0,
                  "gemm_tc_grouped: rows must be 16-byte aligned, n_valid <= BN");
  BSRNN_CHECK_ARG(tiles_per_step > 0 && seq_inner > 0 && tokens_per_sample > 0, "gemm_tc_grouped: bad row map");
  GemmTcArgs a{};
  a.A = reinterpret_cast<const __half*>(A);
  a.W = reinterpret_cast<const __half*>(W);
  a.bias = bias; a.out = out; a.stats = stats; a.ldo = ldo; a.tokens_per_sample = tokens_per_sample;
  a.m_tiles = m_tiles * n_groups; a.n_tiles = 1; a.kcores = kc_max; a.BN = BN; a.n_valid = n_valid;
  a.rows = RowMap{tiles_per_step, R, seq_inner, seq_outer, seq_inner_stride, step_stride};
  a.stats_inner = 1; a.no_resid = 1; a.groups = groups; a.n_groups = n_groups;
  return launch_tc<EPI_RESID_TMA>(a, (cudaStream_t)stream);
}

extern "C" int bsrnn_gemm_tc(const void* A, const void* W, const float* bias, void* out, double* stats,
                               int m_tiles, int n_tiles, int kcores, int BN, int epilogue, long ldo, int n_valid,
                               int out_kcores, long tokens_per_sample, int tiles_per_step, int R, long seq_inner,
                               long seq_outer, long seq_inner_stride, long step_stride, void* stream) {
  return bsrnn_gemm_tc_ex(A, W, bias, out, stats, m_tiles, n_tiles, kcores, BN, epilogue, ldo, n_valid, out_kcores,
                          tokens_per_sample, tiles_per_step, R, seq_inner, seq_outer, seq_inner_stride, step_stride, 1, 0, stream);
}

extern "C" int bsrnn_lstm_step_tc(const void* A, const void* W, const void* gx, float* cstate, void* out_h, int m_tiles,
                                  int n_tiles, int BN, int H, long ld_gx, void* stream) {
  BSRNN_CHECK_ARG(A && W && gx && cstate && out_h, "lstm_step_tc: null pointer");
  BSRNN_CHECK_ARG(m_tiles > 0 && n_tiles > 0 && H > 0 && H % 8 == 0 && BN % 32 == 0 && BN >= 32 && BN <= 256 &&
                  (long)n_tiles * BN >= 4L * H && ld_gx >= 4L * H && ld_gx % 8 == 0, "lstm_step_tc: bad dims");
  GemmTcArgs a{};
  a.A = reinterpret_cast<const __half*>(A);
  a.W = reinterpret_cast<const __half*>(W);
  a.bias = nullptr; a.out = out_h; a.stats = nullptr; a.ldo = 0; a.tokens_per_sample = 1;
  a.m_tiles = m_tiles; a.n_tiles = n_tiles; a.kcores = (H + 15) / 16 * 2; a.BN = BN; a.n_valid = 4 * H; a.out_kcores = (H + 15) / 16 * 2;
  a.gx = reinterpret_cast<const __half*>(gx); a.cstate = cstate; a.ld_gx = ld_gx; a.H = H;
  a.rows = RowMap{m_tiles, m_tiles * 128, 1L << 40, 0, 1, 0};
  return launch_tc<EPI_LSTM_STEP>(a, (cudaStream_t)stream);
}

extern "C" int bsrnn_blstm_step_tc(const void* A_f, const void* W_f, const void* gx_f, float* c_f, void* out_f,
                                   const void* A_b, const void* W_b, const void* gx_b, float* c_b, void* out_b, int m_tiles,
                                   int n_tiles, int BN, int H, long ld_gx, void* stream) {
  BSRNN_CHECK_ARG(A_f && W_f && gx_f && c_f && out_f && A_b && W_b && gx_b && c_b && out_b, "blstm_step_tc: null pointer");
  BSRNN_CHECK_ARG(m_tiles > 0 && n_tiles > 0 && H > 0 && H % 8 == 0 && BN % 32 == 0 && BN >= 32 && BN <= 256 &&
                  (long)n_tiles * BN >= 4L * H && ld_gx >= 4L * H && ld_gx % 8 == 0, "blstm_step_tc: bad dims");
  GemmTcArgs a{};
  a.A = reinterpret_cast<const __half*>(A_f); a.W = reinterpret_cast<const __half*>(W_f);
  a.A2 = reinterpret_cast<const __half*>(A_b); a.W2 = reinterpret_cast<const __half*>(W_b);
  a.bias = nullptr; a.out = out_f; a.out2 = out_b; a.stats = nullptr; a.ldo = 0; a.tokens_per_sample = 1;
  a.m_tiles = 2 * m_tiles; a.dir_tiles = m_tiles; a.n_tiles = n_tiles; a.kcores = (H + 15) / 16 * 2; a.BN = BN; a.n_valid = 4 * H;
  a.out_kcores = (H + 15) / 16 * 2;
  a.gx = reinterpret_cast<const __half*>(gx_f); a.gx2 = reinterpret_cast<const __half*>(gx_b);
  a.cstate = c_f; a.cstate2 = c_b; a.ld_gx = ld_gx; a.H = H;
  a.rows = RowMap{2 * m_tiles, 2 * m_tiles * 128, 1L << 40, 0, 1, 0};
  return launch_tc<EPI_LSTM_STEP>(a, (cudaStream_t)stream);
}

extern "C" int bsrnn_gemm_tc_scaled(const void* A, const void* W, const float* bias, void* out, int m_tiles, int n_tiles,
                                    int kcores, int BN, long ldo, int n_valid, float out_scale, const float* out_scale_ptr,
                                    int ksplit, int tiles_per_step, int R, long seq_inner, long seq_outer,
                                    long seq_inner_stride, long step_stride, void* stream) {
  BSRNN_CHECK_ARG(A && W && out, "gemm_tc_scaled: null pointer");
  BSRNN_CHECK_ARG(m_tiles > 0 && n_tiles > 0 && kcores > 0 && kcores % 2 == 0, "gemm_tc_scaled: bad tile counts (kcores=%d)", kcores);
  BSRNN_CHECK_ARG(BN >= 16 && BN <= 256 && BN % 16 == 0, "gemm_tc_scaled: BN=%d must be a multiple of 16 in [16,256]", BN);
  BSRNN_CHECK_ARG(tiles_per_step > 0 && seq_inner > 0 && n_valid % 4 == 0 && ldo % 4 == 0, "gemm_tc_scaled: bad row map / strides");
  GemmTcArgs a{};
  a.A = reinterpret_cast<const __half*>(A);
  a.W = reinterpret_cast<const __half*>(W);
  a.bias = bias; a.out = out; a.stats = nullptr; a.ldo = ldo; a.tokens_per_sample = 1;
  a.m_tiles = m_tiles; a.n_tiles = n_tiles; a.kcores = kcores; a.BN = BN; a.n_valid = n_valid; a.out_kcores = 0;
  a.out_scale = out_scale; a.out_scale_ptr = out_scale_ptr;
  a.ksplit = 1; a.kps = kcores; a.m_log = m_tiles;
  if (ksplit > 1) {
    BSRNN_CHECK_ARG(bias == nullptr, "gemm_tc_scaled: split-K has no bias epilogue");
    const int kps = ((kcores + ksplit - 1) / ksplit + TC_KS - 1) / TC_KS * TC_KS;
    a.kps = kps;
    a.ksplit = (kcores + kps - 1) / kps;
    a.m_tiles = m_tiles * a.ksplit;
  }
  a.rows = RowMap{tiles_per_step, R, seq_inner, seq_outer, seq_inner_stride, step_stride};
  return launch_tc<EPI_RESID_F32>(a, (cudaStream_t)stream);
}

extern "C" int bsrnn_blstm_step_train_tc(const void* A_f, const void* W_f, void* gx_f, const float* cprev_f, float* cout_f,
                                         void* out_f, const void* A_b, const void* W_b, void* gx_b, const float* cprev_b,
                                         float* cout_b, void* out_b, int m_tiles, int n_tiles, int BN, int H, long ld_gx,
                                         void* stream) {
  BSRNN_CHECK_ARG(A_f && W_f && gx_f && cout_f && out_f && A_b && W_b && gx_b && cout_b && out_b, "blstm_step_train_tc: null pointer");
  BSRNN_CHECK_ARG(m_tiles > 0 && n_tiles > 0 && H > 0 && H % 8 == 0 && BN % 32 == 0 && BN >= 32 && BN <= 256 &&
                  (long)n_tiles * BN >= 4L * H && ld_gx >= 4L * H && ld_gx % 8 == 0, "blstm_step_train_tc: bad dims");
  GemmTcArgs a{};
  a.A = reinterpret_cast<const __half*>(A_f); a.W = reinterpret_cast<const __half*>(W_f);
  a.A2 = reinterpret_cast<const __half*>(A_b); a.W2 = reinterpret_cast<const __half*>(W_b);
  a.bias = nullptr; a.out = out_f; a.out2 = out_b; a.stats = nullptr; a.ldo = 0; a.tokens_per_sample = 1;
  a.m_tiles = 2 * m_tiles; a.dir_tiles = m_tiles; a.n_tiles = n_tiles; a.kcores = (H + 15) / 16 * 2; a.BN = BN; a.n_valid = 4 * H;
  a.out_kcores = (H + 15) / 16 * 2;
  a.gx = reinterpret_cast<const __half*>(gx_f); a.gx2 = reinterpret_cast<const __half*>(gx_b);
  a.cstate = const_cast<float*>(cprev_f); a.cstate2 = const_cast<float*>(cprev_b);
  a.cstate_out = cout_f; a.cstate_out2 = cout_b; a.save_gates = 1;
  a.ld_gx = ld_gx; a.H = H;
  a.rows = RowMap{2 * m_tiles, 2 * m_tiles * 128, 1L << 40, 0, 1, 0};
  return launch_tc<EPI_LSTM_STEP>(a, (cudaStream_t)stream);
}

extern "C" int bsrnn_blstm_bwd_step_tc(const void* A_f, const void* W_f, const void* sg_f, const void* dy_f, const float* ccur_f,
                                       const float* cprev_f, float* dc_f, void* out_f, const void* A_b, const void* W_b,
                                       const void* sg_b, const void* dy_b, const float* ccur_b, const float* cprev_b, float* dc_b,
                                       void* out_b, int m_tiles, int n_tiles, int BN, int H, long ld_sg, long ld_dy,
                                       int valid_rows, void* stream) {
  BSRNN_CHECK_ARG(A_f && W_f && sg_f && dy_f && ccur_f && dc_f && out_f && A_b && W_b && sg_b && dy_b && ccur_b && dc_b && out_b,
                  "blstm_bwd_step_tc: null pointer");
  BSRNN_CHECK_ARG(m_tiles > 0 && n_tiles > 0 && H > 0 && H % 8 == 0 && (4 * H / 8) % 2 == 0 && BN % 32 == 0 && BN >= 32 && BN <= 256 &&
                  (long)n_tiles * BN >= H && ld_sg >= 4L * H && ld_sg % 8 == 0 && ld_dy >= H && ld_dy % 8 == 0 && valid_rows > 0,
                  "blstm_bwd_step_tc: bad dims");
  GemmTcArgs a{};
  a.A = reinterpret_cast<const __half*>(A_f); a.W = reinterpret_cast<const __half*>(W_f);
  a.A2 = reinterpret_cast<const __half*>(A_b); a.W2 = reinterpret_cast<const __half*>(W_b);
  a.bias = nullptr; a.out = out_f; a.out2 = out_b; a.stats = nullptr; a.ldo = 0; a.tokens_per_sample = 1;
  a.m_tiles = 2 * m_tiles; a.dir_tiles = m_tiles; a.n_tiles = n_tiles; a.kcores = 4 * H / 8; a.BN = BN; a.n_valid = H;
  a.out_kcores = 4 * H / 8;
  a.gx = reinterpret_cast<const __half*>(sg_f); a.gx2 = reinterpret_cast<const __half*>(sg_b); a.ld_gx = ld_sg;
  a.dy = reinterpret_cast<const __half*>(dy_f); a.dy2 = reinterpret_cast<const __half*>(dy_b); a.ld_dy = ld_dy;
  a.c_cur = ccur_f; a.c_cur2 = ccur_b; a.c_prev = cprev_f; a.c_prev2 = cprev_b;
  a.cstate = dc_f; a.cstate2 = dc_b; a.H = H; a.valid_rows = valid_rows;
  a.rows = RowMap{2 * m_tiles, 2 * m_tiles * 128, 1L << 40, 0, 1, 0};
  return launch_tc<EPI_LSTM_BWD>(a, (cudaStream_t)stream);
}

extern "C" int bsrnn_blstm_train_fwd_tc(const void* zero_tile, void* y_f, void* y_b, const void* W_f, const void* W_b,
                                        void* gates, float* c_f, float* c_b, int steps, int tiles, int n_tiles, int BN, int H,
                                        void* stream) {
  BSRNN_CHECK_ARG(zero_tile && y_f && y_b && W_f && W_b && gates && c_f && c_b && steps > 0 && tiles > 0,
                  "blstm_train_fwd_tc: bad arguments");
  const size_t kc = (size_t)((H + 15) / 16 * 2);
  const size_t y_step = (size_t)tiles * kc * 1024;
  const size_t g_step = (size_t)tiles * 128 * 8 * H;
  const size_t c_step = (size_t)tiles * 128 * H;
  __half* yf = reinterpret_cast<__half*>(y_f);
  __half* yb = reinterpret_cast<__half*>(y_b);
  __half* g = reinterpret_cast<__half*>(gates);
  for (int s = 0; s < steps; ++s) {
    const int pf = s, pb = steps - 1 - s;
    const int rc = bsrnn_blstm_step_train_tc(
        s == 0 ? zero_tile : (const void*)(yf + (size_t)(pf - 1) * y_step), W_f, g + (size_t)pf * g_step,
        s == 0 ? nullptr : c_f + (size_t)(pf - 1) * c_step, c_f + (size_t)pf * c_step, yf + (size_t)pf * y_step,
        s == 0 ? zero_tile : (const void*)(yb + (size_t)(pb + 1) * y_step), W_b, g + (size_t)pb * g_step + 4 * (size_t)H,
        s == 0 ? nullptr : c_b + (size_t)(pb + 1) * c_step, c_b + (size_t)pb * c_step, yb + (size_t)pb * y_step, tiles, n_tiles,
        BN, H, 8L * H, stream);
    if (rc) return rc;
  }
  return 0;
}

extern "C" int bsrnn_blstm_train_bwd_tc(const void* zero_tile, void* dG_f, void* dG_b, const void* WT_f, const void* WT_b,
                                        const void* gates, const void* dy, const float* c_f, const float* c_b, float* dc_f,
                                        float* dc_b, int steps, int tiles, int n_tiles, int BN, int H, int valid_rows,
                                        void* stream) {
  BSRNN_CHECK_ARG(zero_tile && dG_f && dG_b && WT_f && WT_b && gates && dy && c_f && c_b && dc_f && dc_b && steps > 0 && tiles > 0,
                  "blstm_train_bwd_tc: bad arguments");
  const size_t dg_step = (size_t)tiles * (4 * H / 8) * 1024;
  const size_t g_step = (size_t)tiles * 128 * 8 * H;
  const size_t dy_step = (size_t)tiles * 128 * 2 * H;
  const size_t c_step = (size_t)tiles * 128 * H;
  __half* df = reinterpret_cast<__half*>(dG_f);
  __half* db = reinterpret_cast<__half*>(dG_b);
  const __half* g = reinterpret_cast<const __half*>(gates);
  const __half* dyh = reinterpret_cast<const __half*>(dy);
  for (int sb = 0; sb < steps; ++sb) {
    const int pf = steps - 1 - sb, pb = sb;
    const int rc = bsrnn_blstm_bwd_step_tc(
        sb == 0 ? zero_tile : (const void*)(df + (size_t)(pf + 1) * dg_step), WT_f, g + (size_t)pf * g_step,
        dyh + (size_t)pf * dy_step, c_f + (size_t)pf * c_step, pf > 0 ? c_f + (size_t)(pf - 1) * c_step : nullptr, dc_f,
        df + (size_t)pf * dg_step,
        sb == 0 ? zero_tile : (const void*)(db + (size_t)(pb - 1) * dg_step), WT_b, g + (size_t)pb * g_step + 4 * (size_t)H,
        dyh + (size_t)pb * dy_step + H, c_b + (size_t)pb * c_step, pb < steps - 1 ? c_b + (size_t)(pb + 1) * c_step : nullptr, dc_b,
        db + (size_t)pb * dg_step, tiles, n_tiles, BN, H, 8L * H, 2L * H, valid_rows, stream);
    if (rc) return rc;
  }
  return 0;
}
```

### urgent2026_challenge_track1_b200/runtime_tc.py

```python
from __future__ import annotations

import torch

from . import _lib as L
from .runtime import region, _f64, keepalive

import os

BIG = 1 << 60
_LSTM_SLOTS = {"time": 3, "freq": 3}
for _kv in os.environ.get("BSRNN_LSTM_SLOTS", "").split(","):
    if "=" in _kv:
        _ax, _sv = _kv.split("=")
        _LSTM_SLOTS[_ax] = int(_sv)
LSTM_SCHED = os.environ.get("BSRNN_LSTM_SCHED", "flag")
_FLAG_SLOTS = {"time": 0, "freq": 0}
for _kv in os.environ.get("BSRNN_LSTM_FLAG_SLOTS", "").split(","):
    if "=" in _kv:
        _ax, _sv = _kv.split("=")
        _FLAG_SLOTS[_ax] = int(_sv)
FUSED_AXES = tuple(a for a in os.environ.get("BSRNN_LSTM_FUSED", "time,freq").split(",") if a in ("time", "freq"))
FUSED_GEO = os.environ.get("BSRNN_LSTM_FUSED_GEO", "auto")


GEO14_MAX_PTILES = int(os.environ.get("BSRNN_LSTM_GEO14_MAX_PTILES", "3"))


def _passes(ptiles, groups, slots):
    best = None
    for s in range(1, min(slots, ptiles) + 1):
        gpd = (ptiles + s - 1) // s
        t = ((2 * gpd + groups - 1) // groups) * max(2.3, float(s))
        if best is None or t < best - 1e-9:
            best = t
    return best


def fused_geometry(tiles):
    if FUSED_GEO in ("7", "8", "14"):
        return int(FUSED_GEO)
    ptiles = (tiles + 1) // 2
    if ptiles <= GEO14_MAX_PTILES:
        return 14
    return 7 if 1.08 * _passes(ptiles, 10, 3) < _passes(ptiles, 9, 3) - 1e-9 else 8


_FUSED_SLOTS = {"time": 0, "freq": 0}
for _kv in os.environ.get("BSRNN_LSTM_FUSED_SLOTS", "").split(","):
    if "=" in _kv:
        _ax, _sv = _kv.split("=")
        _FUSED_SLOTS[_ax] = int(_sv)
FC_EPI = L.TC_RESID_F32 if os.environ.get("BSRNN_FC_EPI", "tma") == "ldst" else L.TC_RESID_TMA
CL, LU, LBN, LKC = 8, 49, 208, 50
LGC = LBN // 8
GATE_SCALE = (0.5, 0.5, 1.0, 0.5)


def to_kb8(w, rows_per_tile, kcores):
    rows, K = w.shape
    n_tiles = (rows + rows_per_tile - 1) // rows_per_tile
    buf = torch.zeros(n_tiles * rows_per_tile, kcores * 8, dtype=torch.float32, device=w.device)
    buf[:rows, :K] = w
    return buf.view(n_tiles, rows_per_tile, kcores, 8).permute(0, 2, 1, 3).contiguous().to(torch.float16)


def from_kb8(t, rows, K):
    n_tiles, kcores, rpt, _ = t.shape
    return t.permute(0, 2, 1, 3).reshape(n_tiles * rpt, kcores * 8)[:rows, :K].float()


def _gate_perm(H, dev):
    idx = torch.full((CL, LBN), -1, dtype=torch.long, device=dev)
    for q in range(CL):
        u = torch.arange(LU, device=dev)
        for g in range(4):
            idx[q, 4 * u + g] = g * H + LU * q + u
    return idx


def pack_lstm_tc(rnn):
    H, N = rnn.weight_hh_l0.shape[1], rnn.weight_ih_l0.shape[1]
    if H != CL * LU:
        raise NotImplementedError(f"tensor-core BLSTM kernel is specialised for H=392, got H={H}")
    dev = rnn.weight_hh_l0.device
    perm = _gate_perm(H, dev)
    gsc = torch.tensor(GATE_SCALE, device=dev).repeat(LU)
    gsc = torch.cat([gsc, torch.zeros(LBN - 4 * LU, device=dev)])
    kc_in = (N + 15) // 16 * 2
    one_col = N if (N % 4 == 0 and N < kc_in * 8) else -1
    wih_rows, bih_rows, whh = [], [], []
    for sfx in ("", "_reverse"):
        wi = getattr(rnn, "weight_ih_l0" + sfx).float()
        wh = getattr(rnn, "weight_hh_l0" + sfx).float()
        b = (getattr(rnn, "bias_ih_l0" + sfx) + getattr(rnn, "bias_hh_l0" + sfx)).float()
        for q in range(CL):
            sel = perm[q].clamp_min(0)
            valid = ((perm[q] >= 0).float() * gsc)[:, None]
            wrow = wi[sel] * valid
            brow = b[sel] * valid[:, 0]
            if one_col >= 0:
                wrow = torch.cat([wrow, torch.zeros(wrow.shape[0], kc_in * 8 - N, device=dev)], 1)
                wrow[:, one_col] = brow
            wih_rows.append(wrow)
            bih_rows.append(brow)
            whh.append(to_kb8(wh[sel] * valid, LBN, LKC)[0])
    wih = to_kb8(torch.cat(wih_rows, 0), LBN, kc_in)
    whh = torch.stack(whh).view(2, CL, LKC, LBN, 8).contiguous()
    out = dict(wih=wih, bih=torch.cat(bih_rows).contiguous(), whh=whh, kc_in=kc_in, H=H, N=N, one_col=one_col)
    if one_col >= 0:
        wf = torch.cat([wih.view(2, CL, kc_in, LBN, 8), whh], 2)
        out["wfused"] = wf.view(2, CL, kc_in + LKC, 2, LBN // 2, 8).permute(0, 1, 3, 2, 4, 5).contiguous()
        out["_rnn"] = rnn
    return out


def fused_weights(w, geo):
    if geo == 8:
        return w["wfused"]
    key = f"wfused{geo}"
    if key not in w:
        P, U = (7, 56) if geo == 7 else (14, 28)
        w[key] = pack_lstm_fused7(w["_rnn"], w["kc_in"], w["one_col"], P=P, U=U)
    return w[key]


def pack_lstm_fused7(rnn, kc_in, one_col, P=7, U=56):
    H, N = rnn.weight_hh_l0.shape[1], rnn.weight_ih_l0.shape[1]
    dev = rnn.weight_hh_l0.device
    ul = torch.arange(U, device=dev)
    gsc = torch.tensor(GATE_SCALE, device=dev).repeat(U)[:, None]
    packs = []
    for sfx in ("", "_reverse"):
        wi = getattr(rnn, "weight_ih_l0" + sfx).float()
        wh = getattr(rnn, "weight_hh_l0" + sfx).float()
        b = (getattr(rnn, "bias_ih_l0" + sfx) + getattr(rnn, "bias_hh_l0" + sfx)).float()
        for q in range(P):
            rows = (torch.arange(4, device=dev)[None, :] * H + (U * q + ul)[:, None]).reshape(-1)
            w = torch.zeros(rows.numel(), (kc_in + LKC) * 8, device=dev)
            w[:, :N] = wi[rows]
            w[:, one_col] = b[rows]
            w[:, kc_in * 8: kc_in * 8 + H] = wh[rows]
            w = w * gsc
            packs.append(w.view(2, rows.numel() // 2, kc_in + LKC, 8).permute(0, 2, 1, 3))
    return torch.stack(packs).view(2, P, 2, kc_in + LKC, 2 * U, 8).contiguous().to(torch.float16)


def pack_fc_tc(fc, H):
    N = fc.weight.shape[0]
    BN = (N + 15) // 16 * 16
    w = torch.zeros(N, 2 * LKC * 8, device=fc.weight.device)
    w[:, :H] = fc.weight[:, :H]
    w[:, LKC * 8: LKC * 8 + H] = fc.weight[:, H:]
    bias = torch.zeros(BN, device=w.device)
    bias[:N] = fc.bias
    return dict(w=to_kb8(w, BN, 2 * LKC), b=bias, BN=BN, N=N)


def pack_dual_path_tc(mod):
    layers = []
    for i in range(mod.num_layer):
        e = {}
        for axis in ("time", "freq"):
            norm, rnn, fc = getattr(mod, f"norm_{axis}")[i], getattr(mod, f"rnn_{axis}")[i], getattr(mod, f"fc_{axis}")[i]
            p = pack_lstm_tc(rnn)
            p.update(gamma=norm.weight.float().contiguous(), beta=norm.bias.float().contiguous(), eps=float(norm.eps),
                     fc=pack_fc_tc(fc, p["H"]))
            e[axis] = p
        layers.append(e)
    return layers


class TcWorkspace:

    def __init__(self, B, T, K, N, dev):
        self.key = (B, T, K, N, str(dev))
        M = B * T * K
        self.m_tiles = (M + 127) // 128
        self.tiles_time = (B * K + 127) // 128
        self.tiles_freq = (B * T + 127) // 128
        kc_in = (N + 15) // 16 * 2
        ntile = max(T * self.tiles_time, K * self.tiles_freq)
        self.xhat = torch.empty(ntile * kc_in * 128 * 8, dtype=torch.float16, device=dev)
        self.gates = torch.empty(ntile * 2 * CL * LGC * 128 * 8, dtype=torch.float16, device=dev)
        self.zero_tile = torch.zeros(LKC * 128 * 8, dtype=torch.float16, device=dev)
        self.y = torch.zeros(ntile * 2 * LKC * 128 * 8, dtype=torch.float16, device=dev)
        self.stats = torch.zeros(B, 2, dtype=torch.float64, device=dev)
        self.scale = torch.empty(B, N, dtype=torch.float32, device=dev)
        self.shift = torch.empty(B, N, dtype=torch.float32, device=dev)
        self.counts = _f64([float(T) * K * N], dev)
        self.sync = torch.zeros(max(L.lib().bsrnn_blstm_tc_sync_bytes(), L.lib().bsrnn_blstm_fused_sync_bytes()) // 4,
                                dtype=torch.int32, device=dev)
        self.nbytes = sum(t.numel() * t.element_size() for t in (self.xhat, self.gates, self.y))


_WS = {}
WS_BUDGET_BYTES = int(os.environ.get("BSRNN_WS_BUDGET_GB", "64")) << 30


def workspace(B, T, K, N, dev):
    key = (B, T, K, N, str(dev))
    ws = _WS.pop(key, None)
    if ws is None:
        ws = TcWorkspace(B, T, K, N, dev)
        while _WS and sum(w.nbytes for w in _WS.values()) + ws.nbytes > WS_BUDGET_BYTES:
            _WS.pop(next(iter(_WS)))
    _WS[key] = ws
    return ws


_EXACT_STATS = os.environ.get("BSRNN_TC_EXACT_STATS", "0") == "1"


def dual_path_tc(skip, layers, t_emb=None, max_clusters=0, stats_ready=False, band_stats=None):
    B, T, K, N = skip.shape
    dev = skip.device
    st = L.stream_ptr()
    ws = workspace(B, T, K, N, dev)
    keepalive(ws)
    M = B * T * K
    if not stats_ready:
        L.call("bsrnn_gn_stats", skip.data_ptr(), ws.stats.data_ptr(), B, T * K, N, N, st)
    for i, lay in enumerate(layers):
        for axis in ("time", "freq"):
            last = band_stats is not None and FC_EPI == L.TC_RESID_TMA and i == len(layers) - 1 and axis == "freq"
            w = lay[axis]
            extra = t_emb[i] if (t_emb is not None and axis == "time") else None
            if axis == "time":
                R, steps, tiles, addr = B * K, T, ws.tiles_time, (K, T * K, 1, K)
            else:
                R, steps, tiles, addr = B * T, K, ws.tiles_freq, (1, K, 0, 1)
            with region("norm"):
                L.call("bsrnn_gn_finalize", ws.stats.data_ptr(), w["gamma"].data_ptr(), w["beta"].data_ptr(), L.ptr(extra),
                       ws.scale.data_ptr(), ws.shift.data_ptr(), B, N, ws.counts.data_ptr(), w["eps"], 1, st)
                L.call("bsrnn_norm_cast_kb8_ones", skip.data_ptr(), ws.scale.data_ptr(), ws.shift.data_ptr(),
                       ws.xhat.data_ptr(), N, 0, N, w["kc_in"], steps * tiles, tiles, R, *addr, T * K, 1, w["one_col"], st)
            if axis in FUSED_AXES and "wfused" in w:
                with region(f"lstm_{axis}"):
                    geo = fused_geometry(tiles)
                    if geo in (7, 14):
                        L.call(f"bsrnn_blstm_fused{geo}_tc", ws.xhat.data_ptr(), fused_weights(w, geo).data_ptr(),
                               ws.zero_tile.data_ptr(), ws.y.data_ptr(), R, steps, tiles, max_clusters, _FUSED_SLOTS[axis],
                               ws.sync.data_ptr(), st)
                    else:
                        L.call("bsrnn_blstm_fused_tc", ws.xhat.data_ptr(), w["wfused"].data_ptr(), ws.zero_tile.data_ptr(),
                               ws.y.data_ptr(), R, steps, tiles, max_clusters, _FUSED_SLOTS[axis], ws.sync.data_ptr(), st)
            else:
                with region("inproj"):
                    L.call("bsrnn_gemm_tc", ws.xhat.data_ptr(), w["wih"].data_ptr(),
                           None if w["one_col"] >= 0 else w["bih"].data_ptr(), ws.gates.data_ptr(), None,
                           steps * tiles, 2 * CL, w["kc_in"], LBN, L.TC_F16_KB8, 0, 2 * CL * LBN, 2 * CL * LGC, T * K,
                           tiles, R, *addr, st)
                with region(f"lstm_{axis}"):
                    if LSTM_SCHED == "flag":
                        L.call("bsrnn_blstm_recurrence_tc_flag", ws.gates.data_ptr(), w["whh"].data_ptr(),
                               ws.zero_tile.data_ptr(), ws.y.data_ptr(), R, steps, tiles, max_clusters, _FLAG_SLOTS[axis],
                               ws.sync.data_ptr(), st)
                    else:
                        L.call("bsrnn_blstm_recurrence_tc_ex", ws.gates.data_ptr(), w["whh"].data_ptr(),
                               ws.zero_tile.data_ptr(), ws.y.data_ptr(), R, steps, tiles, max_clusters, _LSTM_SLOTS[axis], st)
            with region("fc"):
                ws.stats.zero_()
                fc = w["fc"]
                L.call("bsrnn_gemm_tc_ex", ws.y.data_ptr(), fc["w"].data_ptr(), fc["b"].data_ptr(), skip.data_ptr(),
                       band_stats.data_ptr() if last else ws.stats.data_ptr(), steps * tiles, 1, 2 * LKC, fc["BN"], FC_EPI,
                       N, N, 0, T * K, tiles, R, *addr, K if last else 1, 0, st)
                if _EXACT_STATS:
                    ws.stats.zero_()
                    L.call("bsrnn_gn_stats", skip.data_ptr(), ws.stats.data_ptr(), B, T * K, N, N, st)
    return band_stats is not None and FC_EPI == L.TC_RESID_TMA


BAND_SPLIT_TC = os.environ.get("BSRNN_BAND_SPLIT_TC", "1") == "1"
BAND_SPLIT_GROUPED = os.environ.get("BSRNN_BAND_SPLIT_GROUPED", "1") == "1"


def pack_band_split_tc(bs):
    K = len(bs.subbands)
    N = bs.fc[0].weight.shape[0]
    dev = bs.fc[0].weight.device
    BN = (N + 15) // 16 * 16
    kcs = [((2 * s + 15) // 16) * 2 for s in bs.subbands]
    w = [to_kb8(bs.fc[k].weight[:, :, 0].float(), BN, kcs[k]).reshape(-1) for k in range(K)]
    w_off, tot = [], 0
    for k in range(K):
        w_off.append(tot)
        tot += w[k].numel()
    bias = torch.zeros(K, BN, device=dev)
    for k in range(K):
        bias[k, :N] = bs.fc[k].bias
    return dict(w=torch.cat(w).contiguous(), w_off=w_off, bias=bias, kcs=kcs, BN=BN, N=N)


def band_split_tc(spec, plan, bs_pack, bs_tc, N, stats):
    from .runtime import _i32, _const_table
    B, T, F, _ = spec.shape
    dev = spec.device
    K = plan.K
    cmax = bs_pack["cmax"]
    st = L.stream_ptr()
    ws = workspace(B, T, K, N, dev)
    keepalive(ws)
    counts = _f64([2.0 * plan.subbands[k] * T for k in range(K)], dev)
    scale = torch.empty(B * K, cmax, dtype=torch.float32, device=dev)
    shift = torch.empty_like(scale)
    L.call("bsrnn_gn_finalize", stats.data_ptr(), bs_pack["gamma"].data_ptr(), bs_pack["beta"].data_ptr(), None,
           scale.data_ptr(), shift.data_ptr(), B * K, cmax, counts.data_ptr(), bs_pack["eps"], K, st)
    tiles = (B * T + 127) // 128
    offs, tot = [], 0
    for k in range(K):
        offs.append(tot)
        tot += tiles * bs_tc["kcs"][k] * 1024
    a_off_d = _const_table(offs, torch.int64, dev)
    xhat = torch.empty(tot, dtype=torch.float16, device=dev)
    wid = _i32([2 * w for w in plan.width], dev)
    bin0 = _i32(list(plan.bin0), dev)
    L.call("bsrnn_band_norm_cast_kb8", spec.data_ptr(), scale.data_ptr(), shift.data_ptr(), xhat.data_ptr(),
           bs_pack["c_off"].data_ptr(), bin0.data_ptr(), wid.data_ptr(), a_off_d.data_ptr(), K, B * T, T, 2 * F, cmax, st)
    out = torch.empty(B, T, K, N, dtype=torch.float32, device=dev)
    ws.stats.zero_()
    if BAND_SPLIT_GROUPED and bs_tc["BN"] >= N:
        desc = []
        for k in range(K):
            desc += [offs[k], bs_tc["w_off"][k], k * N, k * bs_tc["BN"], bs_tc["kcs"][k]]
        groups = _const_table(desc, torch.int64, dev)
        L.call("bsrnn_gemm_tc_grouped", xhat.data_ptr(), bs_tc["w"].data_ptr(), bs_tc["bias"].data_ptr(), out.data_ptr(),
               ws.stats.data_ptr(), groups.data_ptr(), K, tiles, max(bs_tc["kcs"][:K]), bs_tc["BN"], K * N, N, T, tiles,
               B * T, BIG, 0, 1, 0, st)
        return out
    for k in range(K):
        L.call("bsrnn_gemm_tc_ex", xhat.data_ptr() + 2 * offs[k], bs_tc["w"].data_ptr() + 2 * bs_tc["w_off"][k],
               bs_tc["bias"][k].data_ptr(), out.data_ptr() + 4 * k * N, ws.stats.data_ptr(), tiles, 1, bs_tc["kcs"][k],
               bs_tc["BN"], L.TC_RESID_TMA, K * N, N, 0, T, tiles, B * T, BIG, 0, 1, 0, 1, 1, st)
    return out


MASKDEC_ONES = os.environ.get("BSRNN_MASKDEC_ONES", "1") == "1"
MASKDEC_SMS = int(os.environ.get("BSRNN_MASKDEC_SMS", "0"))
MASKDEC_SHARED_NORM = os.environ.get("BSRNN_MASKDEC_SHARED_NORM", "1") == "1"


def pack_mask_decoder_tc(md):
    out = {}
    for name in ("mlp_mask", "mlp_residual"):
        mlps = getattr(md, name)
        N = mlps[0][1].weight.shape[1]
        kc1 = (N + 15) // 16 * 2
        H4 = 4 * N
        kc2 = (H4 + 15) // 16 * 2
        nt1 = (H4 + LBN - 1) // LBN
        w1, b1, w2, b2, bn2 = [], [], [], [], []
        one_col = N if (MASKDEC_ONES and N % 4 == 0 and kc1 * 8 > N) else -1
        for k, m in enumerate(mlps):
            wk = m[1].weight[:, :, 0].float()
            if one_col >= 0:
                bk = m[1].bias.float()
                if MASKDEC_SHARED_NORM:
                    bk = bk + wk @ m[0].bias.float()
                    wk = wk * m[0].weight.float()[None, :]
                wk = torch.cat([wk, bk[:, None]], 1)
            w1.append(to_kb8(wk, LBN, kc1))
            bb = torch.zeros(nt1 * LBN, device=m[1].bias.device); bb[:H4] = m[1].bias
            b1.append(bb)
            w = m[3].weight[:, :, 0].float()
            half = w.shape[0] // 2
            order = torch.stack([torch.arange(half), torch.arange(half) + half], 1).reshape(-1).to(w.device)
            BN = (w.shape[0] + 15) // 16 * 16
            w2.append(to_kb8(w[order], BN, kc2))
            bb = torch.zeros(BN, device=w.device); bb[: w.shape[0]] = m[3].bias[order]
            b2.append(bb)
            bn2.append(BN)
        out[name] = dict(gamma=torch.stack([m[0].weight for m in mlps]).float().contiguous(),
                         beta=torch.stack([m[0].bias for m in mlps]).float().contiguous(),
                         w1=w1, b1=b1, w2=w2, b2=b2, bn2=bn2, kc1=kc1, kc2=kc2, nt1=nt1, N=N, one_col=one_col,
                         shared_norm=bool(MASKDEC_SHARED_NORM and one_col >= 0),
                         eps=float(mlps[0][0].eps))
    return out


def mask_decoder_tc(skip, plan, md_pack, band_stats=None):
    from .runtime import _decoder_norm_tables
    B, T, K, N = skip.shape
    F = plan.F
    dev = skip.device
    st = L.stream_ptr()
    names = ("mlp_residual", "mlp_mask")
    shared = (all(md_pack[n]["shared_norm"] for n in names) and len({md_pack[n]["eps"] for n in names}) == 1
              and len({(md_pack[n]["kc1"], md_pack[n]["one_col"]) for n in names}) == 1)
    if shared:
        ones = _ones_pack(K, N, dev, md_pack[names[0]]["eps"])
        tabs = _decoder_norm_tables(skip, {"shared": ones}, stats=band_stats)
        tabs = {n: tabs["shared"] for n in names}
    else:
        tabs = _decoder_norm_tables(skip, md_pack, stats=band_stats)
    tiles = (B * T + 127) // 128
    outs = {}
    main = torch.cuda.current_stream()
    side = _side_stream(dev)
    fork = torch.cuda.Event()
    capturing = torch.cuda.is_current_stream_capturing()
    bufs = {}
    xshared = None
    for name in names:
        p = md_pack[name]
        if xshared is None or not shared:
            xshared = torch.empty(K * tiles * p["kc1"] * 1024, dtype=torch.float16, device=dev)
        bufs[name] = (xshared,
                      torch.empty(tiles * p["kc2"] * 1024, dtype=torch.float16, device=dev),
                      torch.empty(B, T, F, 2, dtype=torch.float32, device=dev))
    with region("maskdec"):
        if shared:
            p = md_pack[names[0]]
            scale, shift = tabs[names[0]][0], tabs[names[0]][1]
            L.call("bsrnn_norm_cast_kb8_ones", skip.data_ptr(), scale.data_ptr(), shift.data_ptr(), xshared.data_ptr(), N, 0, N,
                   p["kc1"], K * tiles, tiles, B * T, 1, K, 0, 1, T * K, K, p["one_col"], st)
        fork.record(main)
        side.wait_event(fork)
        prev_limit = L.lib().bsrnn_gemm_tc_limit_ctas(MASKDEC_SMS)
        for name, stream in (("mlp_residual", side), ("mlp_mask", main)):
            p = md_pack[name]
            scale, shift = tabs[name][0], tabs[name][1]
            xhat, hidden, o = bufs[name]
            with torch.cuda.stream(stream):
                st = L.stream_ptr()
                if not shared:
                    L.call("bsrnn_norm_cast_kb8_ones", skip.data_ptr(), scale.data_ptr(), shift.data_ptr(), xhat.data_ptr(), N, 0,
                           N, p["kc1"], K * tiles, tiles, B * T, 1, K, 0, 1, T * K, K, p["one_col"], st)
                for k in range(K):
                    L.call("bsrnn_gemm_tc", xhat.data_ptr() + 2 * k * tiles * p["kc1"] * 1024, p["w1"][k].data_ptr(),
                           None if p["one_col"] >= 0 else p["b1"][k].data_ptr(), hidden.data_ptr(), None, tiles, p["nt1"],
                           p["kc1"], LBN, L.TC_TANH_KB8,
                           0, 4 * N, p["kc2"], B * T, tiles, B * T, BIG, 0, 1, 0, st)
                    L.call("bsrnn_gemm_tc", hidden.data_ptr(), p["w2"][k].data_ptr(), p["b2"][k].data_ptr(),
                           o.data_ptr() + 8 * plan.bin0[k], None, tiles, 1, p["kc2"], p["bn2"][k], L.TC_GLU_F32, 2 * F,
                           2 * plan.width[k], 0, B * T, tiles, B * T, BIG, 0, 1, 0, st)
            if stream is side and not capturing:
                for t in (xhat, hidden, o, skip, scale, shift):
                    t.record_stream(side)
            outs[name] = o
        L.lib().bsrnn_gemm_tc_limit_ctas(prev_limit)
        main.wait_stream(side)
    return outs["mlp_mask"], outs["mlp_residual"]


_SIDE = {}
_ONES = {}


def _ones_pack(K, N, dev, eps):
    key = (K, N, str(dev), eps)
    t = _ONES.get(key)
    if t is None:
        t = _ONES[key] = dict(gamma=torch.ones(K, N, device=dev), beta=torch.zeros(K, N, device=dev), eps=eps)
    return t


def _side_stream(dev):
    key = str(dev)
    if key not in _SIDE:
        _SIDE[key] = torch.cuda.Stream(device=dev)
    return _SIDE[key]
```

Before: 5723.

## Fuse mask decoder MLPs into one persistent 2-CTA tensor-core kernel

Replaces the per-band pair of GEMM launches (tanh hidden GEMM then GLU output GEMM) for both mask and residual heads, previously split across two streams, with a single persistent cluster kernel. The hidden activations stay in shared memory and TMEM chunk by chunk instead of round-tripping through global memory, and weights for both heads are packed into one buffer with a per-band descriptor table. The norm's affine terms are always folded into the first-layer weights. It also removes the L2-hint, reverse-M and CTA-limit experiment knobs from the generic GEMM. The new kernel limits kc1 to 32, requires both heads to have the same widths, and adds a warp-specialized pipeline whose scheduling across CTA pairs must balance well.

```diff
diff --git a/include/bsrnn_b200.h b/include/bsrnn_b200.h
--- a/include/bsrnn_b200.h
+++ b/include/bsrnn_b200.h
@@ -61,7 +61,8 @@
                           const long long* groups, int n_groups, int m_tiles, int kc_max, int BN, long ldo, int n_valid,
                           long tokens_per_sample, int tiles_per_step, int R, long seq_inner, long seq_outer,
                           long seq_inner_stride, long step_stride, void* stream);
-int bsrnn_gemm_tc_limit_ctas(int n);
+int bsrnn_mask_decoder_tc(const void* z, const void* w, const float* bias, const int32_t* desc, float* mask, float* resid,
+                          long ldo, int K, int tiles, int R, int kc1, int kc2, void* stream);
 int bsrnn_band_norm_cast_kb8(const float* spec, const float* scale, const float* shift, void* out, const int32_t* c_off,
                              const int32_t* bin0, const int32_t* width2, const long long* a_off, int K, long rows, int T,
                              int F2, int cmax, void* stream);
diff --git a/urgent2026_challenge_track1_b200/_lib.py b/urgent2026_challenge_track1_b200/_lib.py
--- a/urgent2026_challenge_track1_b200/_lib.py
+++ b/urgent2026_challenge_track1_b200/_lib.py
@@ -37,7 +37,8 @@
                          c_int, c_int, c_long, c_int, c_int, c_long, c_long, c_long, c_long, c_int, c_int, c_void_p],
     "bsrnn_gemm_tc_grouped": [c_void_p, c_void_p, c_void_p, c_void_p, c_void_p, c_void_p, c_int, c_int, c_int, c_int, c_long,
                               c_int, c_long, c_int, c_int, c_long, c_long, c_long, c_long, c_void_p],
-    "bsrnn_gemm_tc_limit_ctas": [c_int],
+    "bsrnn_mask_decoder_tc": [c_void_p, c_void_p, c_void_p, c_void_p, c_void_p, c_void_p, c_long, c_int, c_int, c_int, c_int,
+                              c_int, c_void_p],
     "bsrnn_blstm_fused_train_tc": [c_int, c_void_p, c_void_p, c_void_p, c_void_p, c_void_p, c_long, c_void_p, c_void_p, c_void_p,
                                    c_void_p, c_int, c_int, c_int, c_int, c_int, c_void_p, c_void_p],
     "bsrnn_blstm_fused_train_scratch_bytes": [c_int, c_int],
diff --git a/urgent2026_challenge_track1_b200/csrc/gemm_tc.cu b/urgent2026_challenge_track1_b200/csrc/gemm_tc.cu
--- a/urgent2026_challenge_track1_b200/csrc/gemm_tc.cu
+++ b/urgent2026_challenge_track1_b200/csrc/gemm_tc.cu
@@ -75,8 +75,6 @@
   alignas(64) CUtensorMap tmap;
   const long long* groups;
   int n_groups;
-  int l2_keep;
-  int reverse_m;
   int m_inner;
   int use_tmap;
   int tm_col_step;
@@ -369,19 +367,14 @@
     m = (int)blockIdx.x / n_tiles;
     dm = (int)gridDim.x / n_tiles;
     dn = resident ? 0 : (int)gridDim.x - dm * n_tiles;
-    if (a.reverse_m && n_tiles == 1 && !resident) {
-      rev = true;
-      m = m_tiles - 1 - (int)blockIdx.x;
-      dm = -(int)gridDim.x;
-    } else if (a.m_inner > 1 && !resident && dn == 0) {
+    if (a.m_inner > 1 && !resident && dn == 0) {
       inner = a.m_inner; tps = a.rows.tiles_per_step;
       lin = m;
       m = (lin % inner) * tps + lin / inner;
     }
   }
-  bool rev = false;
   int inner = 0, tps = 0, lin = 0;
-  __device__ __forceinline__ bool valid() const { return rev ? m >= 0 : (inner ? lin < m_tiles : m < m_tiles); }
+  __device__ __forceinline__ bool valid() const { return inner ? lin < m_tiles : m < m_tiles; }
   __device__ __forceinline__ void next() {
     if (inner) {
       lin += dm;
@@ -510,10 +503,9 @@
             const uint32_t slice = (uint32_t)nk * 2048 / (uint32_t)a.mc;
             bulk_g2s_multicast(sA + stage * a_stage_bytes + crank * slice, gA + (size_t)kc0 * 2048 + crank * slice, slice,
                                full + stage, cmask);
-          } else if (a.l2_keep & 2)
-            bulk_g2s_hint(sA + stage * a_stage_bytes, gA + (size_t)kc0 * 2048, nk * 2048, full + stage, l2_policy_evict_last());
-          else
-          bulk_g2s(sA + stage * a_stage_bytes, gA + (size_t)kc0 * 2048, nk * 2048, full + stage);
+          } else {
+            bulk_g2s(sA + stage * a_stage_bytes, gA + (size_t)kc0 * 2048, nk * 2048, full + stage);
+          }
           if (!a.b_resident)
             bulk_g2s(sB + stage * b_stage_bytes, gB + (size_t)kc0 * BN * 16, nk * BN * 16, full + stage);
           if (++stage == NST) { stage = 0; phase ^= 1; }
@@ -602,10 +594,7 @@
         store_kb8_cores_smem<2>(my_stg + 12 * 2048, v3);
         fence_proxy_async_shared();
         named_bar_sync(bar_id, 128);
-        if (leader && do_store && nA) {
-          if (EPI == EPI_TANH_KB8 && (a.l2_keep & 1)) bulk_s2g_hint(gdst, stg, nA * 2048, l2_policy_evict_last());
-          else bulk_s2g(gdst, stg, nA * 2048);
-        }
+        if (leader && do_store && nA) bulk_s2g(gdst, stg, nA * 2048);
         tmem_ld_x32(t_row + 112, v0);
         tmem_ld_x32(t_row + 144, v1);
         tmem_ld_x32(t_row + 176, v2);
@@ -623,10 +612,7 @@
         else store_kb8_cores_smem<3>(my_stg + 8 * 2048, v2);
         fence_proxy_async_shared();
         named_bar_sync(bar_id, 128);
-        if (leader && do_store && nB) {
-          if (EPI == EPI_TANH_KB8 && (a.l2_keep & 1)) bulk_s2g_hint(gdst + 14 * 2048, stg, nB * 2048, l2_policy_evict_last());
-          else bulk_s2g(gdst + 14 * 2048, stg, nB * 2048);
-        }
+        if (leader && do_store && nB) bulk_s2g(gdst + 14 * 2048, stg, nB * 2048);
       }
       if (leader) bulk_store_wait_all();
     } else if constexpr (EPI == EPI_RESID_TMA) {
@@ -888,14 +874,6 @@
   return (size_t)128 * ldr * 4;
 }
 
-static int g_cta_limit = 0;
-
-static bool tanh_bulk_enabled() {
-  static int v = -1;
-  if (v < 0) { const char* e = getenv("BSRNN_TANH_BULK"); v = (e && e[0] == '0') ? 0 : 1; }
-  return v != 0;
-}
-
 template <int EPI>
 static int launch_tc(GemmTcArgs a, cudaStream_t st) {
   static int sms = 0;
@@ -919,16 +897,6 @@
       a.b_resident = 1;
       if (mc_env > 1 && a.n_tiles % mc_env == 0) step_mc = mc_env;
     }
-  }
-  if (EPI == EPI_GLU_F32) {
-    static int rev_env = -1;
-    if (rev_env < 0) { const char* e = getenv("BSRNN_GLU_REVERSE"); rev_env = (e && e[0] == '0') ? 0 : 1; }
-    a.reverse_m = rev_env;
-  }
-  if (EPI == EPI_TANH_KB8 || EPI == EPI_GLU_F32) {
-    static int keep_env = -1;
-    if (keep_env < 0) { const char* e = getenv("BSRNN_HIDDEN_L2"); keep_env = (e && e[0] == '1') ? 1 : 0; }
-    a.l2_keep = keep_env ? (EPI == EPI_TANH_KB8 ? 1 : 2) : 0;
   }
   const size_t extra_smem = EPI == EPI_RESID_TMA ? tc_resbuf_bytes(a.BN, a.n_valid) + 128 : 0;
   if (EPI == EPI_RESID_TMA) {
@@ -982,11 +950,10 @@
     smem_set = smem;
   }
   const int total = a.m_tiles * a.n_tiles;
-  const int sms_use = (g_cta_limit > 0 && g_cta_limit < sms) ? g_cta_limit : sms;
-  int grid = total < sms_use ? total : sms_use;
+  int grid = total < sms ? total : sms;
   if (a.b_resident) {
     const int nt_all = a.n_tiles * (a.dir_tiles > 0 ? 2 : 1);
-    grid = (sms_use / nt_all) * nt_all;
+    grid = (sms / nt_all) * nt_all;
     if (grid < nt_all) grid = nt_all;
     if (a.dir_tiles > 0) a.pf_dist = 0;
   }
@@ -1027,7 +994,7 @@
     a.mc = 1;
     gemm_tc_kernel<EPI_F16_KB8, 208><<<grid, tc_threads(EPI_F16_KB8), smem_ip, st>>>(a);
   } else if (EPI == EPI_TANH_KB8 && a.BN == 208 && a.kcores == 26 && a.bias == nullptr && a.b_resident &&
-             a.out_kcores > (a.n_tiles - 1) * 26 && tanh_bulk_enabled()) {
+             a.out_kcores > (a.n_tiles - 1) * 26) {
     a.stages = 5;
     a.mc = 1;
     const size_t smem_ip = tc_smem_bytes(a.BN, a.kcores, true, false, a.stages) + 2 * 14 * 2048;
@@ -1104,12 +1071,6 @@
   set_error("gemm_tc: unknown epilogue %d", epilogue);
   return 1;
 }
-extern "C" int bsrnn_gemm_tc_limit_ctas(int n) {
-  const int prev = g_cta_limit;
-  g_cta_limit = n > 0 ? n : 0;
-  return prev;
-}
-
 extern "C" int bsrnn_gemm_tc_grouped(const void* A, const void* W, const float* bias, void* out, double* stats,
                                        const long long* groups, int n_groups, int m_tiles, int kc_max, int BN, long ldo,
                                        int n_valid, long tokens_per_sample, int tiles_per_step, int R, long seq_inner,
diff --git a/urgent2026_challenge_track1_b200/csrc/maskdec.cu b/urgent2026_challenge_track1_b200/csrc/maskdec.cu
--- /dev/null
+++ b/urgent2026_challenge_track1_b200/csrc/maskdec.cu
@@ -0,0 +1,383 @@
+#include "common.cuh"
+#include "umma.cuh"
+#include <cuda_fp16.h>
+
+namespace bsrnn {
+using namespace umma;
+
+namespace md {
+constexpr int HC = 16;
+constexpr int KS1 = 16, KS2 = 8;
+constexpr int STAGES = 6;
+constexpr uint32_t STAGE_BYTES = 16384;
+constexpr uint32_t H_BYTES = HC * 2048;
+constexpr int EPI_WARPS = 8;
+constexpr int THREADS = (2 + EPI_WARPS) * 32;
+constexpr int D2_COL = 256;
+constexpr int DESC = 8;
+constexpr int MAX_KC1 = 32;
+__host__ __device__ constexpr size_t smem_bytes(int kc1) {
+  return (size_t)kc1 * 2048 + 2 * H_BYTES + STAGES * STAGE_BYTES + 256;
+}
+}
+
+struct MaskDecArgs {
+  const __half* z;
+  const __half* w;
+  const float* bias;
+  const int* desc;
+  float* out0;
+  float* out1;
+  long ldo;
+  int K, tiles, R, kc1, kc2;
+};
+
+__device__ __forceinline__ float md_tanh(float x) {
+  float y;
+  asm("tanh.approx.f32 %0, %1;" : "=f"(y) : "f"(x));
+  return y;
+}
+__device__ __forceinline__ float md_sigmoid(float x) { return fmaf(md_tanh(0.5f * x), 0.5f, 0.5f); }
+__device__ __forceinline__ uint32_t md_pack_h2(float a, float b) {
+  __half2 v = __floats2half2_rn(a, b);
+  return *reinterpret_cast<uint32_t*>(&v);
+}
+
+__global__ void __launch_bounds__(md::THREADS, 1) maskdec_kernel(const __grid_constant__ MaskDecArgs a) {
+  using namespace md;
+  extern __shared__ __align__(128) uint8_t smem[];
+  uint8_t* sZ = smem;
+  uint8_t* sH = smem + (size_t)a.kc1 * 2048;
+  uint8_t* sW = sH + 2 * H_BYTES;
+  uint64_t* bars = reinterpret_cast<uint64_t*>(sW + STAGES * STAGE_BYTES);
+  uint64_t* full = bars;
+  uint64_t* empty = full + STAGES;
+  uint64_t* pfull = empty + STAGES;
+  uint64_t* z_full = pfull + STAGES;
+  uint64_t* pz_full = z_full + 1;
+  uint64_t* z_empty = pz_full + 1;
+  uint64_t* d1_full = z_empty + 1;
+  uint64_t* d1_empty = d1_full + 2;
+  uint64_t* h_full = d1_empty + 2;
+  uint64_t* h_empty = h_full + 2;
+  uint64_t* d2_full = h_empty + 2;
+  uint64_t* d2_empty = d2_full + 1;
+  uint32_t* tmem_slot = reinterpret_cast<uint32_t*>(d2_empty + 1);
+
+  const int warp = threadIdx.x >> 5, lane = threadIdx.x & 31;
+  const uint32_t e = cluster_ctarank() & 1u;
+  const uint32_t leader = 0;
+  if (threadIdx.x == 0) {
+    for (int i = 0; i < STAGES; ++i) { mbar_init(full + i, 1); mbar_init(empty + i, 1); mbar_init(pfull + i, 1); }
+    mbar_init(z_full, 1); mbar_init(pz_full, 1); mbar_init(z_empty, 1);
+    for (int i = 0; i < 2; ++i) {
+      mbar_init(d1_full + i, 1); mbar_init(d1_empty + i, 2 * EPI_WARPS);
+      mbar_init(h_full + i, 2 * EPI_WARPS); mbar_init(h_empty + i, 1);
+    }
+    mbar_init(d2_full, 1); mbar_init(d2_empty, 2 * EPI_WARPS);
+    fence_barrier_init();
+  }
+  if (warp == 2) tmem_alloc2(tmem_slot, 512);
+  tc_fence_before();
+  __syncthreads();
+  cluster_sync();
+  tc_fence_after();
+  const uint32_t tmem_base = *tmem_slot;
+
+  const int npairs = (a.tiles + 1) / 2;
+  const int items = a.K * npairs;
+  const int pair = (int)cluster_id_x(), npair_grid = (int)num_clusters_x();
+  const int nch = (a.kc2 + HC - 1) / HC;
+  const int nz1 = (a.kc1 + KS1 - 1) / KS1;
+
+  if (warp == 0) {
+    if (elect_one()) {
+      uint32_t stage = 0, phase = 0, zph = 0;
+      const uint8_t* gz = reinterpret_cast<const uint8_t*>(a.z);
+      const uint8_t* gw = reinterpret_cast<const uint8_t*>(a.w);
+      const uint32_t zbytes = (uint32_t)a.kc1 * 2048;
+      auto z_src = [&](int it) {
+        const int k = it / npairs, jp = it - k * npairs;
+        int j = 2 * jp + (int)e;
+        if (j >= a.tiles) j = a.tiles - 1;
+        return gz + ((size_t)k * a.tiles + j) * zbytes;
+      };
+      auto load_stage = [&](const uint8_t* src, uint32_t bytes) {
+        mbar_wait(empty + stage, phase ^ 1);
+        mbar_expect_tx(full + stage, bytes);
+        bulk_g2s(sW + stage * STAGE_BYTES, src, bytes, full + stage);
+        if (++stage == STAGES) { stage = 0; phase ^= 1; }
+      };
+      for (int it = pair; it < items; it += npair_grid) {
+        const int k = it / npairs;
+        mbar_wait(z_empty, zph ^ 1);
+        zph ^= 1;
+        mbar_expect_tx(z_full, zbytes);
+        const uint8_t* zs = z_src(it);
+        for (uint32_t off = 0; off < zbytes; off += 32768) bulk_g2s(sZ + off, zs + off, min(32768u, zbytes - off), z_full);
+        if (it + npair_grid < items) bulk_prefetch_l2(z_src(it + npair_grid), zbytes);
+        for (int f = 0; f < 2; ++f) {
+          const int* D = a.desc + (f * a.K + k) * DESC;
+          const long w1 = __ldg(D), w2 = __ldg(D + 1);
+          const int bn2 = __ldg(D + 4);
+          auto g1 = [&](int c) {
+            const int n1 = 8 * min(HC, a.kc2 - HC * c);
+            const uint8_t* src = gw + 2 * (w1 + (long)c * a.kc1 * 1024 + (long)e * a.kc1 * (n1 / 2) * 8);
+            for (int s = 0; s < nz1; ++s) {
+              const int nk = min(KS1, a.kc1 - KS1 * s);
+              load_stage(src + (size_t)s * KS1 * (n1 / 2) * 16, (uint32_t)nk * (n1 / 2) * 16);
+            }
+          };
+          auto g2 = [&](int c) {
+            const int nc = min(HC, a.kc2 - HC * c);
+            const uint8_t* src = gw + 2 * (w2 + (long)HC * c * bn2 * 8 + (long)e * nc * (bn2 / 2) * 8);
+            for (int s = 0; s * KS2 < nc; ++s) {
+              const int nk = min(KS2, nc - KS2 * s);
+              load_stage(src + (size_t)s * KS2 * (bn2 / 2) * 16, (uint32_t)nk * (bn2 / 2) * 16);
+            }
+          };
+          for (int c = 0; c < nch; ++c) {
+            g1(c);
+            if (c > 0) g2(c - 1);
+          }
+          g2(nch - 1);
+        }
+      }
+    }
+  } else if (warp == 1) {
+    if (e == 0) {
+      if (elect_one()) {
+        uint32_t stage = 0, phase = 0, zph = 0, d2ph = 0;
+        uint32_t n1cnt = 0, hcnt = 0;
+        const uint16_t pair_mask = 3;
+        auto next_stage = [&]() {
+          mbar_wait(full + stage, phase);
+          mbar_wait(pfull + stage, phase);
+          tc_fence_after();
+        };
+        auto release_stage = [&]() {
+          mma_commit2_multicast(empty + stage, pair_mask);
+          if (++stage == STAGES) { stage = 0; phase ^= 1; }
+        };
+        for (int it = pair; it < items; it += npair_grid) {
+          const int k = it / npairs;
+          mbar_wait(z_full, zph);
+          mbar_wait(pz_full, zph);
+          zph ^= 1;
+          tc_fence_after();
+          for (int f = 0; f < 2; ++f) {
+            const int bn2 = __ldg(a.desc + (f * a.K + k) * DESC + 4);
+            const uint32_t idesc2 = idesc_f16_f32(256, (uint32_t)bn2);
+            auto g1 = [&](int c) {
+              const int n1 = 8 * min(HC, a.kc2 - HC * c);
+              const uint32_t b = n1cnt & 1;
+              mbar_wait(d1_empty + b, ((n1cnt >> 1) & 1) ^ 1);
+              tc_fence_after();
+              const uint32_t idesc1 = idesc_f16_f32(256, (uint32_t)n1);
+              const uint64_t da0 = smem_desc_kb8(smem_u32(sZ), 2048, 128);
+              for (int s = 0; s < nz1; ++s) {
+                const int nk = min(KS1, a.kc1 - KS1 * s);
+                next_stage();
+                const uint64_t da = da0 + (uint64_t)((s * KS1 * 2048) >> 4);
+                const uint64_t db = smem_desc_kb8(smem_u32(sW + stage * STAGE_BYTES), (uint32_t)(n1 / 2) * 16, 128);
+                for (int j = 0; j < nk / 2; ++j)
+                  mma_f16_ss_2cta(tmem_base + b * 128, da + (uint64_t)((j * 2 * 2048) >> 4), db + (uint64_t)((j * 2 * (n1 / 2) * 16) >> 4),
+                                  idesc1, (s | j) != 0);
+                release_stage();
+              }
+              mma_commit2_multicast(d1_full + b, pair_mask);
+              if (f == 1 && c == nch - 1) mma_commit2_multicast(z_empty, pair_mask);
+              ++n1cnt;
+            };
+            auto g2 = [&](int c) {
+              const int nc = min(HC, a.kc2 - HC * c);
+              const uint32_t hb = hcnt & 1;
+              if (c == 0) {
+                mbar_wait(d2_empty, d2ph ^ 1);
+                d2ph ^= 1;
+              }
+              mbar_wait_cluster(h_full + hb, (hcnt >> 1) & 1);
+              tc_fence_after();
+              const uint64_t da0 = smem_desc_kb8(smem_u32(sH + hb * H_BYTES), 2048, 128);
+              for (int s = 0; s * KS2 < nc; ++s) {
+                const int nk = min(KS2, nc - KS2 * s);
+                next_stage();
+                const uint64_t da = da0 + (uint64_t)((s * KS2 * 2048) >> 4);
+                const uint64_t db = smem_desc_kb8(smem_u32(sW + stage * STAGE_BYTES), (uint32_t)(bn2 / 2) * 16, 128);
+                for (int j = 0; j < nk / 2; ++j)
+                  mma_f16_ss_2cta(tmem_base + D2_COL, da + (uint64_t)((j * 2 * 2048) >> 4), db + (uint64_t)((j * 2 * (bn2 / 2) * 16) >> 4),
+                                  idesc2, (c | s | j) != 0);
+                release_stage();
+              }
+              mma_commit2_multicast(h_empty + hb, pair_mask);
+              if (c == nch - 1) mma_commit2_multicast(d2_full, pair_mask);
+              ++hcnt;
+            };
+            for (int c = 0; c < nch; ++c) {
+              g1(c);
+              if (c > 0) g2(c - 1);
+            }
+            g2(nch - 1);
+          }
+        }
+      }
+    } else {
+      uint32_t stage = 0, phase = 0, zph = 0;
+      int per_item = 0;
+      for (int c = 0; c < nch; ++c) per_item += nz1 + (min(HC, a.kc2 - HC * c) + KS2 - 1) / KS2;
+      per_item *= 2;
+      for (int it = pair; it < items; it += npair_grid) {
+        mbar_wait(z_full, zph);
+        zph ^= 1;
+        if (lane == 0) mbar_arrive_cluster_relaxed(pz_full, leader);
+        __syncwarp();
+        for (int i = 0; i < per_item; ++i) {
+          mbar_wait(full + stage, phase);
+          if (lane == 0) mbar_arrive_cluster_relaxed(pfull + stage, leader);
+          __syncwarp();
+          if (++stage == STAGES) { stage = 0; phase ^= 1; }
+        }
+      }
+    }
+  } else {
+    const int q = warp & 3, half = (warp - 2) >> 2;
+    const int r = q * 32 + lane;
+    const uint32_t t_lane = tmem_base + ((uint32_t)(q * 32) << 16);
+    uint32_t n1cnt = 0, hcnt = 0, d2ph = 0;
+    for (int it = pair; it < items; it += npair_grid) {
+      const int k = it / npairs, jp = it - k * npairs;
+      const int j = 2 * jp + (int)e;
+      const int seq = j * 128 + r;
+      const bool row_ok = j < a.tiles && seq < a.R;
+      for (int f = 0; f < 2; ++f) {
+        const int* D = a.desc + (f * a.K + k) * DESC;
+        const int b1_off = __ldg(D + 2), b2_off = __ldg(D + 3), bn2 = __ldg(D + 4), col0 = __ldg(D + 5), ncols = __ldg(D + 6);
+        for (int c = 0; c < nch; ++c, ++n1cnt, ++hcnt) {
+          const int n1 = 8 * min(HC, a.kc2 - HC * c);
+          const int mine = max(0, min(64, n1 - 64 * half));
+          const uint32_t b = n1cnt & 1;
+          float bl0 = 0.f, bl1 = 0.f;
+          if (b1_off >= 0) {
+            const float* bp = a.bias + b1_off + HC * 8 * c + 64 * half;
+            if (lane < mine) bl0 = __ldg(bp + lane);
+            if (32 + lane < mine) bl1 = __ldg(bp + 32 + lane);
+          }
+          uint32_t v0[32], v1[32];
+          mbar_wait(d1_full + b, (n1cnt >> 1) & 1);
+          tc_fence_after();
+          const uint32_t ta = t_lane + b * 128 + 64 * half;
+          if (mine >= 32) tmem_ld_x32(ta, v0);
+          else if (mine == 16) tmem_ld_x16(ta, reinterpret_cast<uint32_t(&)[16]>(v0));
+          if (mine == 64) tmem_ld_x32(ta + 32, v1);
+          else if (mine == 48) tmem_ld_x16(ta + 32, reinterpret_cast<uint32_t(&)[16]>(v1));
+          tmem_ld_wait();
+          tmem_ld_pin(v0); tmem_ld_pin(v1);
+          tc_fence_before();
+          __syncwarp();
+          if (lane == 0) mbar_arrive_cluster_relaxed(d1_empty + b, leader);
+          if (b1_off >= 0) {
+#pragma unroll
+            for (int i = 0; i < 32; ++i) {
+              v0[i] = __float_as_uint(__uint_as_float(v0[i]) + __shfl_sync(0xffffffffu, bl0, i));
+              v1[i] = __float_as_uint(__uint_as_float(v1[i]) + __shfl_sync(0xffffffffu, bl1, i));
+            }
+          }
+          uint4 pk[8];
+#pragma unroll
+          for (int i = 0; i < 4; ++i) {
+            pk[i] = make_uint4(md_pack_h2(md_tanh(__uint_as_float(v0[8 * i])), md_tanh(__uint_as_float(v0[8 * i + 1]))),
+                               md_pack_h2(md_tanh(__uint_as_float(v0[8 * i + 2])), md_tanh(__uint_as_float(v0[8 * i + 3]))),
+                               md_pack_h2(md_tanh(__uint_as_float(v0[8 * i + 4])), md_tanh(__uint_as_float(v0[8 * i + 5]))),
+                               md_pack_h2(md_tanh(__uint_as_float(v0[8 * i + 6])), md_tanh(__uint_as_float(v0[8 * i + 7]))));
+            pk[4 + i] = make_uint4(md_pack_h2(md_tanh(__uint_as_float(v1[8 * i])), md_tanh(__uint_as_float(v1[8 * i + 1]))),
+                                   md_pack_h2(md_tanh(__uint_as_float(v1[8 * i + 2])), md_tanh(__uint_as_float(v1[8 * i + 3]))),
+                                   md_pack_h2(md_tanh(__uint_as_float(v1[8 * i + 4])), md_tanh(__uint_as_float(v1[8 * i + 5]))),
+                                   md_pack_h2(md_tanh(__uint_as_float(v1[8 * i + 6])), md_tanh(__uint_as_float(v1[8 * i + 7]))));
+          }
+          const uint32_t hb = hcnt & 1;
+          mbar_wait(h_empty + hb, ((hcnt >> 1) & 1) ^ 1);
+          uint8_t* hrow = sH + hb * H_BYTES + (size_t)(8 * half) * 2048 + r * 16;
+#pragma unroll
+          for (int i = 0; i < 8; ++i)
+            if (8 * i < mine) *reinterpret_cast<uint4*>(hrow + i * 2048) = pk[i];
+          fence_proxy_async_shared();
+          __syncwarp();
+          if (lane == 0) mbar_arrive_cluster(h_full + hb, leader);
+        }
+        mbar_wait(d2_full, d2ph);
+        d2ph ^= 1;
+        tc_fence_after();
+        float* orow = (f == 0 ? a.out0 : a.out1) + (long)seq * a.ldo + col0;
+        const int npc = (bn2 + 31) >> 5;
+        for (int p = half; p < npc; p += 2) {
+          const int cnt = min(32, bn2 - 32 * p);
+          const float bl = (lane < cnt) ? __ldg(a.bias + b2_off + 32 * p + lane) : 0.f;
+          uint32_t v[32];
+          if (cnt == 32) tmem_ld_x32(t_lane + D2_COL + 32 * p, v);
+          else tmem_ld_x16(t_lane + D2_COL + 32 * p, reinterpret_cast<uint32_t(&)[16]>(v));
+          tmem_ld_wait();
+          tmem_ld_pin(v);
+#pragma unroll
+          for (int i = 0; i < 32; i += 4) {
+            if (i >= cnt) break;
+            const float g0 = (__uint_as_float(v[i]) + __shfl_sync(0xffffffffu, bl, i)) *
+                             md_sigmoid(__uint_as_float(v[i + 1]) + __shfl_sync(0xffffffffu, bl, i + 1));
+            const float g1 = (__uint_as_float(v[i + 2]) + __shfl_sync(0xffffffffu, bl, i + 2)) *
+                             md_sigmoid(__uint_as_float(v[i + 3]) + __shfl_sync(0xffffffffu, bl, i + 3));
+            const int oc = 16 * p + i / 2;
+            if (row_ok && oc < ncols) *reinterpret_cast<float2*>(orow + oc) = make_float2(g0, g1);
+          }
+        }
+        tc_fence_before();
+        __syncwarp();
+        if (lane == 0) mbar_arrive_cluster_relaxed(d2_empty, leader);
+      }
+    }
+  }
+  tc_fence_before();
+  __syncthreads();
+  cluster_sync();
+  if (warp == 2) {
+    tc_fence_after();
+    tmem_dealloc2(tmem_base, 512);
+  }
+}
+
+}
+using namespace bsrnn;
+
+extern "C" int bsrnn_mask_decoder_tc(const void* z, const void* w, const float* bias, const int32_t* desc, float* mask,
+                                     float* resid, long ldo, int K, int tiles, int R, int kc1, int kc2, void* stream) {
+  BSRNN_CHECK_ARG(z && w && bias && desc && mask && resid, "mask_decoder_tc: null pointer");
+  BSRNN_CHECK_ARG(K > 0 && tiles > 0 && R > 0 && R <= tiles * 128, "mask_decoder_tc: bad shape (K=%d tiles=%d R=%d)", K, tiles, R);
+  BSRNN_CHECK_ARG(kc1 > 0 && kc1 % 2 == 0 && kc1 <= md::MAX_KC1 && kc2 > 0 && kc2 % 2 == 0,
+                  "mask_decoder_tc: kc1=%d must be even and <= %d, kc2=%d even", kc1, md::MAX_KC1, kc2);
+  BSRNN_CHECK_ARG(ldo % 2 == 0 && (reinterpret_cast<uintptr_t>(mask) & 7) == 0 && (reinterpret_cast<uintptr_t>(resid) & 7) == 0,
+                  "mask_decoder_tc: output rows must be 8-byte aligned");
+  static int sms = 0;
+  if (sms == 0) {
+    int dev = 0;
+    cudaGetDevice(&dev);
+    if (cudaDeviceGetAttribute(&sms, cudaDevAttrMultiProcessorCount, dev) != cudaSuccess || sms <= 0) sms = 148;
+  }
+  const size_t smem = md::smem_bytes(kc1);
+  static size_t smem_set = 0;
+  if (smem > smem_set) {
+    BSRNN_CUDA_OK(cudaFuncSetAttribute(maskdec_kernel, cudaFuncAttributeMaxDynamicSharedMemorySize, (int)smem));
+    smem_set = smem;
+  }
+  MaskDecArgs a{};
+  a.z = reinterpret_cast<const __half*>(z); a.w = reinterpret_cast<const __half*>(w); a.bias = bias; a.desc = desc;
+  a.out0 = mask; a.out1 = resid; a.ldo = ldo; a.K = K; a.tiles = tiles; a.R = R; a.kc1 = kc1; a.kc2 = kc2;
+  const int items = K * ((tiles + 1) / 2);
+  const int pairs = items < sms / 2 ? items : sms / 2;
+  cudaLaunchConfig_t cfg = {};
+  cfg.gridDim = dim3(2 * pairs); cfg.blockDim = dim3(md::THREADS); cfg.dynamicSmemBytes = smem; cfg.stream = (cudaStream_t)stream;
+  cudaLaunchAttribute at[1];
+  at[0].id = cudaLaunchAttributeClusterDimension;
+  at[0].val.clusterDim.x = 2; at[0].val.clusterDim.y = 1; at[0].val.clusterDim.z = 1;
+  cfg.attrs = at; cfg.numAttrs = 1;
+  BSRNN_CUDA_OK(cudaLaunchKernelEx(&cfg, maskdec_kernel, a));
+  BSRNN_LAUNCH_OK();
+  return 0;
+}
diff --git a/urgent2026_challenge_track1_b200/runtime_tc.py b/urgent2026_challenge_track1_b200/runtime_tc.py
--- a/urgent2026_challenge_track1_b200/runtime_tc.py
+++ b/urgent2026_challenge_track1_b200/runtime_tc.py
@@ -334,9 +334,41 @@
     return out
 
 
-MASKDEC_ONES = os.environ.get("BSRNN_MASKDEC_ONES", "1") == "1"
-MASKDEC_SMS = int(os.environ.get("BSRNN_MASKDEC_SMS", "0"))
-MASKDEC_SHARED_NORM = os.environ.get("BSRNN_MASKDEC_SHARED_NORM", "1") == "1"
+MD_HC = 16
+
+
+def _pack_maskdec_fused(fams, dev):
+    ws, bs, desc = [], [], []
+    woff = boff = 0
+    for p in fams:
+        kc1, kc2 = p["kc1"], p["kc2"]
+        for k in range(len(p["w1"])):
+            w1 = p["w1"][k].permute(0, 2, 1, 3).reshape(-1, kc1 * 8)[: kc2 * 8]
+            bn2 = p["bn2"][k]
+            w2 = p["w2"][k].permute(0, 2, 1, 3).reshape(bn2, kc2 * 8)
+            parts1, parts2 = [], []
+            for c in range(0, kc2, MD_HC):
+                nc = min(MD_HC, kc2 - c)
+                rows = w1[8 * c: 8 * (c + nc)]
+                for h in range(2):
+                    half1 = rows[h * 4 * nc: (h + 1) * 4 * nc]
+                    parts1.append(half1.reshape(4 * nc, kc1, 8).permute(1, 0, 2).reshape(-1))
+                    half2 = w2[h * bn2 // 2: (h + 1) * bn2 // 2, 8 * c: 8 * (c + nc)]
+                    parts2.append(half2.reshape(bn2 // 2, nc, 8).permute(1, 0, 2).reshape(-1))
+            t1, t2 = torch.cat(parts1), torch.cat(parts2)
+            b1_off = -1
+            if p["one_col"] < 0:
+                b1_off = boff
+                b1 = torch.zeros(kc2 * 8, device=dev)
+                b1[: min(kc2 * 8, p["b1"][k].numel())] = p["b1"][k][: kc2 * 8]
+                bs.append(b1)
+                boff += b1.numel()
+            desc.append([woff, woff + t1.numel(), b1_off, boff, bn2])
+            ws += [t1, t2]
+            woff += t1.numel() + t2.numel()
+            bs.append(p["b2"][k].float())
+            boff += bn2
+    return torch.cat(ws).contiguous(), torch.cat(bs).float().contiguous(), desc
 
 
 def pack_mask_decoder_tc(md):
@@ -349,17 +381,15 @@
         kc2 = (H4 + 15) // 16 * 2
         nt1 = (H4 + LBN - 1) // LBN
         w1, b1, w2, b2, bn2 = [], [], [], [], []
-        one_col = N if (MASKDEC_ONES and N % 4 == 0 and kc1 * 8 > N) else -1
+        one_col = N if (N % 4 == 0 and kc1 * 8 > N) else -1
         for k, m in enumerate(mlps):
             wk = m[1].weight[:, :, 0].float()
+            bk = m[1].bias.float() + wk @ m[0].bias.float()
+            wk = wk * m[0].weight.float()[None, :]
             if one_col >= 0:
-                bk = m[1].bias.float()
-                if MASKDEC_SHARED_NORM:
-                    bk = bk + wk @ m[0].bias.float()
-                    wk = wk * m[0].weight.float()[None, :]
                 wk = torch.cat([wk, bk[:, None]], 1)
             w1.append(to_kb8(wk, LBN, kc1))
-            bb = torch.zeros(nt1 * LBN, device=m[1].bias.device); bb[:H4] = m[1].bias
+            bb = torch.zeros(nt1 * LBN, device=bk.device); bb[:H4] = bk
             b1.append(bb)
             w = m[3].weight[:, :, 0].float()
             half = w.shape[0] // 2
@@ -369,80 +399,47 @@
             bb = torch.zeros(BN, device=w.device); bb[: w.shape[0]] = m[3].bias[order]
             b2.append(bb)
             bn2.append(BN)
-        out[name] = dict(gamma=torch.stack([m[0].weight for m in mlps]).float().contiguous(),
-                         beta=torch.stack([m[0].bias for m in mlps]).float().contiguous(),
-                         w1=w1, b1=b1, w2=w2, b2=b2, bn2=bn2, kc1=kc1, kc2=kc2, nt1=nt1, N=N, one_col=one_col,
-                         shared_norm=bool(MASKDEC_SHARED_NORM and one_col >= 0),
-                         eps=float(mlps[0][0].eps))
+        out[name] = dict(w1=w1, b1=b1, w2=w2, b2=b2, bn2=bn2, kc1=kc1, kc2=kc2, nt1=nt1, N=N, one_col=one_col,
+                         shared_norm=True, eps=float(mlps[0][0].eps))
+    fams = [out["mlp_mask"], out["mlp_residual"]]
+    if len({(p["kc1"], p["kc2"], p["one_col"], p["eps"]) for p in fams}) != 1:
+        raise NotImplementedError("mask decoder families of different widths")
+    w, bias, desc = _pack_maskdec_fused(fams, fams[0]["w1"][0].device)
+    out["fused"] = dict(w=w, bias=bias, desc=desc)
     return out
 
 
 def mask_decoder_tc(skip, plan, md_pack, band_stats=None):
-    from .runtime import _decoder_norm_tables
+    from .runtime import _decoder_norm_tables, _i32
     B, T, K, N = skip.shape
     F = plan.F
     dev = skip.device
     st = L.stream_ptr()
-    names = ("mlp_residual", "mlp_mask")
-    shared = (all(md_pack[n]["shared_norm"] for n in names) and len({md_pack[n]["eps"] for n in names}) == 1
-              and len({(md_pack[n]["kc1"], md_pack[n]["one_col"]) for n in names}) == 1)
-    if shared:
-        ones = _ones_pack(K, N, dev, md_pack[names[0]]["eps"])
-        tabs = _decoder_norm_tables(skip, {"shared": ones}, stats=band_stats)
-        tabs = {n: tabs["shared"] for n in names}
-    else:
-        tabs = _decoder_norm_tables(skip, md_pack, stats=band_stats)
+    p = md_pack["mlp_mask"]
+    fz = md_pack["fused"]
+    if p["kc1"] > 32:
+        raise NotImplementedError(f"tensor-core mask decoder: num_channel {N} > 256")
+    ones = _ones_pack(K, N, dev, p["eps"])
+    scale, shift = _decoder_norm_tables(skip, {"shared": ones}, stats=band_stats)["shared"][:2]
     tiles = (B * T + 127) // 128
-    outs = {}
-    main = torch.cuda.current_stream()
-    side = _side_stream(dev)
-    fork = torch.cuda.Event()
-    capturing = torch.cuda.is_current_stream_capturing()
-    bufs = {}
-    xshared = None
-    for name in names:
-        p = md_pack[name]
-        if xshared is None or not shared:
-            xshared = torch.empty(K * tiles * p["kc1"] * 1024, dtype=torch.float16, device=dev)
-        bufs[name] = (xshared,
-                      torch.empty(tiles * p["kc2"] * 1024, dtype=torch.float16, device=dev),
-                      torch.empty(B, T, F, 2, dtype=torch.float32, device=dev))
+    Kall = len(p["w1"])
+    desc = []
+    for f in range(2):
+        for k in range(K):
+            w1o, w2o, b1o, b2o, bn2 = fz["desc"][f * Kall + k]
+            desc += [w1o, w2o, b1o, b2o, bn2, 2 * plan.bin0[k], 2 * plan.width[k], 0]
+    desc_d = _i32(desc, dev)
+    z = torch.empty(K * tiles * p["kc1"] * 1024, dtype=torch.float16, device=dev)
+    mask = torch.empty(B, T, F, 2, dtype=torch.float32, device=dev)
+    resid = torch.empty(B, T, F, 2, dtype=torch.float32, device=dev)
     with region("maskdec"):
-        if shared:
-            p = md_pack[names[0]]
-            scale, shift = tabs[names[0]][0], tabs[names[0]][1]
-            L.call("bsrnn_norm_cast_kb8_ones", skip.data_ptr(), scale.data_ptr(), shift.data_ptr(), xshared.data_ptr(), N, 0, N,
-                   p["kc1"], K * tiles, tiles, B * T, 1, K, 0, 1, T * K, K, p["one_col"], st)
-        fork.record(main)
-        side.wait_event(fork)
-        prev_limit = L.lib().bsrnn_gemm_tc_limit_ctas(MASKDEC_SMS)
-        for name, stream in (("mlp_residual", side), ("mlp_mask", main)):
-            p = md_pack[name]
-            scale, shift = tabs[name][0], tabs[name][1]
-            xhat, hidden, o = bufs[name]
-            with torch.cuda.stream(stream):
-                st = L.stream_ptr()
-                if not shared:
-                    L.call("bsrnn_norm_cast_kb8_ones", skip.data_ptr(), scale.data_ptr(), shift.data_ptr(), xhat.data_ptr(), N, 0,
-                           N, p["kc1"], K * tiles, tiles, B * T, 1, K, 0, 1, T * K, K, p["one_col"], st)
-                for k in range(K):
-                    L.call("bsrnn_gemm_tc", xhat.data_ptr() + 2 * k * tiles * p["kc1"] * 1024, p["w1"][k].data_ptr(),
-                           None if p["one_col"] >= 0 else p["b1"][k].data_ptr(), hidden.data_ptr(), None, tiles, p["nt1"],
-                           p["kc1"], LBN, L.TC_TANH_KB8,
-                           0, 4 * N, p["kc2"], B * T, tiles, B * T, BIG, 0, 1, 0, st)
-                    L.call("bsrnn_gemm_tc", hidden.data_ptr(), p["w2"][k].data_ptr(), p["b2"][k].data_ptr(),
-                           o.data_ptr() + 8 * plan.bin0[k], None, tiles, 1, p["kc2"], p["bn2"][k], L.TC_GLU_F32, 2 * F,
-                           2 * plan.width[k], 0, B * T, tiles, B * T, BIG, 0, 1, 0, st)
-            if stream is side and not capturing:
-                for t in (xhat, hidden, o, skip, scale, shift):
-                    t.record_stream(side)
-            outs[name] = o
-        L.lib().bsrnn_gemm_tc_limit_ctas(prev_limit)
-        main.wait_stream(side)
-    return outs["mlp_mask"], outs["mlp_residual"]
-
-
-_SIDE = {}
+        L.call("bsrnn_norm_cast_kb8_ones", skip.data_ptr(), scale.data_ptr(), shift.data_ptr(), z.data_ptr(), N, 0, N,
+               p["kc1"], K * tiles, tiles, B * T, 1, K, 0, 1, T * K, K, p["one_col"], st)
+        L.call("bsrnn_mask_decoder_tc", z.data_ptr(), fz["w"].data_ptr(), fz["bias"].data_ptr(), desc_d.data_ptr(),
+               mask.data_ptr(), resid.data_ptr(), 2 * F, K, tiles, B * T, p["kc1"], p["kc2"], st)
+    return mask, resid
+
+
 _ONES = {}
 
 
@@ -452,10 +449,3 @@
     if t is None:
         t = _ONES[key] = dict(gamma=torch.ones(K, N, device=dev), beta=torch.zeros(K, N, device=dev), eps=eps)
     return t
-
-
-def _side_stream(dev):
-    key = str(dev)
-    if key not in _SIDE:
-        _SIDE[key] = torch.cuda.Stream(device=dev)
-    return _SIDE[key]
```

After: 5753, median of 6. Within noise of the previous version (+0.5%).
